# jsappl/DeepPreconditioning

Hardware: NVIDIA B200
Metric: pcg_solves_per_sec (higher is better)
Workload: dtype f64

## Files before the change

deeppreconditioning_b200/_lib.py:

```python

from __future__ import annotations

import ctypes as C
import os
from pathlib import Path

import torch

LIB_PATH = Path(os.environ.get("DPCG_LIB") or Path(__file__).resolve().parent / "lib" / "libdpcg.so")

DP_OK = 0
DP_ERR_STRUCTURE = 5
DP_ERR_TIMEOUT = 6

PRECOND_IDENTITY, PRECOND_JACOBI, PRECOND_MULTIPLY, PRECOND_SOLVE, PRECOND_CSR = range(5)
ENGINE_FUSED, ENGINE_STEPPED = 0, 1
ASSEMBLE_TRIL, ASSEMBLE_TRIL_T, ASSEMBLE_SYMMETRISE = 0, 1, 2

_p = C.c_void_p
_i32 = C.c_int32
_i64 = C.c_int64


class PcgSystem(C.Structure):

    _fields_ = [(name, _i32) for name in (
        "n", "precond", "a_nnz", "m_nnz", "mt_nnz", "fwd_nchunks", "bwd_nchunks",
        "fwd_max_level_chunks", "bwd_max_level_chunks", "solve_algorithm")] + [(name, _p) for name in (
            "a_rowptr", "a_col", "a_val", "m_rowptr", "m_col", "m_val", "mt_rowptr", "mt_col", "mt_val",
            "dinv", "fwd_plan", "bwd_plan",
            "fwd_ls_rowptr", "fwd_ls_col", "fwd_ls_val", "fwd_ls_perm", "fwd_ls_level",
            "bwd_ls_rowptr", "bwd_ls_col", "bwd_ls_val", "bwd_ls_perm", "bwd_ls_level",
            "b", "x", "work", "iters_out", "res_out", "history", "coef",
            "a_col16", "a_val32", "a_tile_base", "m_col16", "m_val32", "m_tile_base",
            "mt_col16", "mt_val32", "mt_tile_base")]


class TrsvSystem(C.Structure):

    _fields_ = [("n", _i32), ("upper", _i32), ("max_level_chunks", _i32), ("reserved", _i32), ("nchunks", _i64)] + [
        (name, _p) for name in ("rowptr", "col", "val", "plan", "b", "x")]


class TrsvLsSystem(C.Structure):

    _fields_ = [("n", _i32), ("nnz", _i32), ("upper", _i32), ("flags", _i32)] + [
        (name, _p) for name in ("rowptr_p", "col_p", "val_p", "perm", "level_sorted", "b", "x")]


class PcgParams(C.Structure):

    _fields_ = [("rtol", C.c_double), ("max_iter", _i32), ("engine", _i32), ("check_every", _i32), ("reserved", _i32)]


class SpconvLayer(C.Structure):

    _fields_ = [("nout", _i64), ("ntaps", _i32), ("cin", _i32), ("cout", _i32), ("reserved", _i32)] + [
        (name, _p) for name in ("src", "in_", "weight", "bias", "slope", "head_weight", "head_bias", "indices", "out")]


class DpcgError(RuntimeError):
    pass


_SIGNATURES = {
    "dp_version": (C.c_int, []),
    "dp_status_string": (C.c_char_p, [C.c_int]),
    "dp_last_cuda_error": (C.c_char_p, []),
    "dp_device_info": (C.c_int, [C.POINTER(C.c_int)] * 3),
    "dp_csr_from_coo_workspace_bytes": (C.c_size_t, [_i32, _i64]),
    "dp_csr_from_coo": (C.c_int, [_p, _p, _i64, _i32, _i32, _i32, _p, _p, _p, _p, _p, _p, C.c_size_t, _p]),
    "dp_csr_transpose_workspace_bytes": (C.c_size_t, [_i32, _i32]),
    "dp_csr_transpose": (C.c_int, [_i32, _i32, _p, _p, _p, _p, _p, _p, _p, C.c_size_t, _p]),
    "dp_csr_inv_diagonal": (C.c_int, [_i32, _p, _p, _p, _p, _p, _p]),
    "dp_csr_aat_nnz": (C.c_int, [_i32, _p, _p, _p, _p, _p, _p]),
    "dp_spmv_csr_f64": (C.c_int, [_i32, _i32, _p, _p, _p, _p, _p, _p]),
    "dp_csr_pack_tile_rows": (_i32, []),
    "dp_csr_pack": (C.c_int, [_i32, _i32, _p, _p, _p, _p, _p, _p, _p, _p]),
    "dp_spmv_csr_packed_f64": (C.c_int, [_i32, _i32, _p, _p, _p, _p, _p, _p, _p]),
    "dp_coo_spmv_batch_f32": (C.c_int, [_p, _p, _i64, _i32, _i32, _p, _i32, _p, _p]),
    "dp_sptrsv_analyse_workspace_bytes": (C.c_size_t, [_i32]),
    "dp_sptrsv_analyse": (C.c_int, [_i32, _p, _p, _i32, _p, _p, _p, _p, _p, _p, C.c_size_t, _p]),
    "dp_sptrsv_plan_chunks": (_i64, [_i32, _p]),
    "dp_sptrsv_plan_sizes_workspace_bytes": (C.c_size_t, [_i32]),
    "dp_sptrsv_plan_sizes": (C.c_int, [_i32, _p, _p, _p, _p, _p, C.c_size_t, _p]),
    "dp_sptrsv_plan_build": (C.c_int, [_i32, _i32, _p, _p, _p, _p, _i64, _p]),
    "dp_sptrsv_workspace_bytes": (C.c_size_t, []),
    "dp_sptrsv_solve_f64": (C.c_int, [_i32, _p, _p, _p, _i32, _p, _i64, _i32, _p, _p, _p, _p, C.c_size_t, _p]),
    "dp_sptrsv_batch_workspace_bytes": (C.c_size_t, [_i32]),
    "dp_sptrsv_solve_batch_f64": (C.c_int, [C.POINTER(TrsvSystem), _i32, _p, _p, C.c_size_t, _p]),
    "dp_sptrsv_permute_workspace_bytes": (C.c_size_t, [_i32]),
    "dp_sptrsv_permute": (C.c_int, [_i32, _i32, _p, _p, _p, _p, _p, _p, _p, _p, _p, _p, _p, C.c_size_t, _p]),
    "dp_sptrsv_ls_limits": (None, [_p]),
    "dp_sptrsv_ls_workspace_bytes": (C.c_size_t, [_i32]),
    "dp_sptrsv_ls_solve_batch_f64": (C.c_int, [C.POINTER(TrsvLsSystem), _i32, _p, C.c_size_t, _p]),
    "dp_sptrsv_ls_prepare": (C.c_int, [C.POINTER(TrsvLsSystem), _i32, _p, C.c_size_t, _p]),
    "dp_sptrsv_ls_launch": (C.c_int, [_i32, _p, C.c_size_t, _p]),
    "dp_sptrsv_ts_prepare": (C.c_int, [C.POINTER(TrsvLsSystem), _i32, _p, C.c_size_t, _p]),
    "dp_sptrsv_ts_launch": (C.c_int, [_i32, _i32, _i32, _i32, _i32, _p, _p, _p]),
    "dp_sptrsv_ts_limits": (None, [_p]),
    "dp_sptrsv_ts_workspace_bytes": (C.c_size_t, [C.POINTER(TrsvLsSystem), _i32]),
    "dp_sptrsv_ts_solve_batch_f64": (C.c_int, [C.POINTER(TrsvLsSystem), _i32, _p, _p, C.c_size_t, _p]),
    "dp_ic0_f64": (C.c_int, [_i32, _p, _p, _p, _p, _p, _i64, _i32, _p, _p, C.c_size_t, _p]),
    "dp_icholt_host": (C.c_int, [_i32, _p, _p, _p, _i32, C.c_double, _p, _p, _p, _i64, _p]),
    "dp_spconv_sort_workspace_bytes": (C.c_size_t, [_i32, _i32]),
    "dp_spconv_sort_sites": (C.c_int, [_p, _i64, _i32, _i32, _i32, _p, _p, _p, _p, _p, C.c_size_t, _p]),
    "dp_spconv_rules_workspace_bytes": (C.c_size_t, [_i32, _i32, _i32]),
    "dp_spconv_rules_count": (C.c_int, [_p, _p, _i32, _i32, _i32, _i32, _i32, _p, _p, C.c_size_t, _p]),
    "dp_spconv_rules_fill": (C.c_int, [_p, _p, _p, _i32, _i32, _i32, _i32, _i32, _p, _p, _p, _p, _p]),
    "dp_spconv_layer_f32": (C.c_int, [C.POINTER(SpconvLayer), _p]),
    "dp_pcg_work_doubles": (_i64, [_i32]),
    "dp_pcg_workspace_bytes": (C.c_size_t, [_i32]),
    "dp_debug_pcg_trace": (C.c_int, [_p, _i32, _p, _i32]),
    "dp_debug_pipe_trace": (C.c_int, [_p, _i32, _i32]),
    "dp_pcg_solve_f64": (C.c_int, [C.POINTER(PcgSystem), _i32, C.POINTER(PcgParams), _p, _p, C.c_size_t, _p]),
}

EXPORTED_SYMBOLS = tuple(_SIGNATURES)

_lib = None


def lib() -> C.CDLL:
    global _lib
    if _lib is None:
        if not LIB_PATH.exists():
            raise DpcgError(
                f"{LIB_PATH} is missing: build it with `python -m deeppreconditioning_b200.build` "
                "(nvcc, sm_100a). deeppreconditioning_b200 has no CPU fallback."
            )
        handle = C.CDLL(str(LIB_PATH))
        for name, (restype, argtypes) in _SIGNATURES.items():
            fn = getattr(handle, name)
            fn.restype, fn.argtypes = restype, argtypes
        _lib = handle
    return _lib


def check(status: int, what: str = "") -> None:
    if status != DP_OK:
        l = lib()
        msg = l.dp_status_string(status).decode()
        if status == 4:
            msg += f" ({l.dp_last_cuda_error().decode()})"
        raise DpcgError(f"libdpcg {what}: {msg}")


def ptr(t: torch.Tensor | None) -> int | None:
    if t is None:
        return None
    if not t.is_cuda:
        raise DpcgError("libdpcg takes device pointers: got a CPU tensor (no CPU fallback)")
    if not t.is_contiguous():
        raise DpcgError("libdpcg needs contiguous tensors")
    return t.data_ptr()


def stream_ptr(device=None) -> int:
    return torch.cuda.current_stream(device).cuda_stream


def device_info() -> dict:
    sm, ctas, l2 = C.c_int(), C.c_int(), C.c_int()
    check(lib().dp_device_info(C.byref(sm), C.byref(ctas), C.byref(l2)), "dp_device_info")
    return {"sm_count": sm.value, "pcg_ctas_per_sm": ctas.value, "l2_bytes": l2.value}


def raise_on_flag(flag: torch.Tensor, what: str) -> None:
    value = int(flag.item())
    if value:
        raise DpcgError(f"libdpcg {what}: device flag {value} ({lib().dp_status_string(value).decode()})")
```

deeppreconditioning_b200/cg.py:

```python

from __future__ import annotations

import ctypes
import time
from dataclasses import dataclass, field

import torch

from . import _lib
from .precond import Identity, _Operator, as_operator, fill_packed
from .sparse import CsrMatrix, _workspace, as_csr, pack_many

_ENGINES = {"fused": _lib.ENGINE_FUSED, "stepped": _lib.ENGINE_STEPPED}


@dataclass
class PcgResult:
    seconds: float
    iterations: int
    info: int
    x_hat: torch.Tensor
    res: float
    history: list = field(default_factory=list)
    alphas: list = field(default_factory=list)
    betas: list = field(default_factory=list)

    @property
    def kappa(self) -> float:
        from .spectrum import kappa_estimate

        return kappa_estimate(self.alphas, self.betas) if self.alphas else float("nan")


def stopping_criterion(_, rk, b):
    return torch.inner(rk, rk) / torch.inner(b, b)


class PcgBatch:

    def __init__(self, systems, rtol: float = 1e-8, max_iter: int = 1024, engine: str = "fused",
                 check_every: int = 32, history: bool = False, device=None, pack: bool = True) -> None:
        if not systems:
            raise ValueError("empty batch")
        self.device = torch.device(device) if device is not None else None
        self.rtol, self.max_iter = float(rtol), int(max_iter)
        self.params = _lib.PcgParams(self.rtol, self.max_iter, _ENGINES[engine], int(check_every), 0)
        self.entries = []
        lib = _lib.lib()
        for item in systems:
            A, b, M = item[0], item[1], item[2]
            x0 = item[3] if len(item) > 3 else None
            A = as_csr(A, self.device)
            if self.device is None:
                self.device = A.device
            if A.device != self.device:
                raise _lib.DpcgError("all systems of a batch must live on one device")
            M = as_operator(M, self.device)
            n = A.n
            b_dev = b.detach().to(device=self.device, dtype=torch.float64).contiguous()
            if b_dev.shape != (n,):
                raise ValueError(f"right-hand side has shape {tuple(b_dev.shape)}, expected ({n},)")
            f64 = dict(dtype=torch.float64, device=self.device)
            x = (x0.detach().to(**f64).clone() if x0 is not None else torch.zeros(n, **f64)).contiguous()
            work = torch.empty(lib.dp_pcg_work_doubles(n), **f64)
            hist = torch.full((self.max_iter + 1,), float("nan"), **f64) if history else None
            coef = torch.full((2 * (self.max_iter + 1),), float("nan"), **f64) if history else None
            self.entries.append(dict(A=A, M=M, b=b_dev, x=x, work=work, hist=hist, coef=coef, out_device=b.device))
        nsys = len(self.entries)
        if any(getattr(e["M"], "tile_stream", False) for e in self.entries):
            self.params = _lib.PcgParams(self.rtol, self.max_iter, _ENGINES["stepped"], min(int(check_every), 8), 0)
        solve_mode = any(e["M"].precond == _lib.PRECOND_SOLVE for e in self.entries)
        if pack and engine == "fused" and not solve_mode:
            pack_many([m for e in self.entries for m in [e["A"], *e["M"].stream_matrices()]])
        self.iters = torch.full((nsys,), -1, dtype=torch.int32, device=self.device)
        self.res = torch.full((nsys,), float("nan"), dtype=torch.float64, device=self.device)
        self.flag = torch.zeros(1, dtype=torch.int32, device=self.device)
        self.ws = _workspace(lib.dp_pcg_workspace_bytes(nsys), self.device)
        self.descs = (_lib.PcgSystem * nsys)()
        for i, e in enumerate(self.entries):
            d, A = self.descs[i], e["A"]
            d.n, d.a_nnz = A.n, A.nnz
            d.a_rowptr, d.a_col, d.a_val = _lib.ptr(A.rowptr), _lib.ptr(A.col), _lib.ptr(A.val)
            fill_packed(d, "a", A)
            e["M"].fill(d)
            if not pack:
                for tag in ("a", "m", "mt"):
                    for name in ("col16", "val32", "tile_base"):
                        setattr(d, f"{tag}_{name}", None)
            d.b, d.x, d.work = _lib.ptr(e["b"]), _lib.ptr(e["x"]), _lib.ptr(e["work"])
            d.iters_out = self.iters.data_ptr() + 4 * i
            d.res_out = self.res.data_ptr() + 8 * i
            d.history = _lib.ptr(e["hist"])
            d.coef = _lib.ptr(e["coef"])

    def __len__(self) -> int:
        return len(self.entries)

    def reset(self, x0s=None) -> None:
        for i, e in enumerate(self.entries):
            if x0s is not None and x0s[i] is not None:
                e["x"].copy_(x0s[i])
            else:
                e["x"].zero_()
        self.iters.fill_(-1)
        self.res.fill_(float("nan"))

    def solve(self) -> None:
        with torch.cuda.device(self.device):
            _lib.check(_lib.lib().dp_pcg_solve_f64(self.descs, len(self.entries), ctypes.byref(self.params),
                                                   _lib.ptr(self.flag), _lib.ptr(self.ws), self.ws.numel(),
                                                   _lib.stream_ptr(self.device)), "dp_pcg_solve_f64")

    def results(self, seconds: float = 0.0) -> list[PcgResult]:
        _lib.raise_on_flag(self.flag, "dp_pcg_solve_f64")
        iters, res = self.iters.cpu().tolist(), self.res.cpu().tolist()
        xs = []
        for e in self.entries:
            if e["out_device"].type == "cpu":
                host = torch.empty(e["x"].shape, dtype=torch.float64, pin_memory=True)
                host.copy_(e["x"], non_blocking=True)
                xs.append(host)
            else:
                xs.append(e["x"].to(e["out_device"]))
        torch.cuda.synchronize(self.device)
        out = []
        for i, e in enumerate(self.entries):
            hist = e["hist"][: iters[i] + 1].cpu().tolist() if e["hist"] is not None and iters[i] >= 0 else []
            alphas, betas = [], []
            if e["coef"] is not None and iters[i] > 0:
                c = e["coef"][: 2 * iters[i]].cpu().view(-1, 2)
                alphas, betas = c[:, 0].tolist(), c[:, 1].tolist()
                betas[0] = 0.0
            out.append(PcgResult(seconds, int(iters[i]), 0, xs[i], float(res[i]), hist, alphas, betas))
        return out


def pcg_solve_batch(systems, rtol: float = 1e-8, max_iter: int = 1024, engine: str = "fused", check_every: int = 32,
                    history: bool = False, device=None, pack: bool = True) -> list[PcgResult]:
    batch = PcgBatch(systems, rtol, max_iter, engine, check_every, history, device, pack)
    torch.cuda.synchronize(batch.device)
    start = time.perf_counter()
    batch.solve()
    torch.cuda.synchronize(batch.device)
    return batch.results(time.perf_counter() - start)


def pcg_solve(A, b, M=None, x0=None, rtol: float = 1e-8, max_iter: int = 1024, engine: str = "fused",
              check_every: int = 32, history: bool = False, pack: bool = True) -> PcgResult:
    return pcg_solve_batch([(A, b, M, x0)], rtol, max_iter, engine, check_every, history, pack=pack)[0]


def preconditioned_conjugate_gradient(A, b: torch.Tensor, M, x0=None, x_true=None, rtol=1e-8, max_iter=1024):
    result = pcg_solve(A, b, M, x0, rtol, max_iter)
    return result.seconds, result.iterations, 0


def conjugate_gradient(A, b, x0=None, x_true=None, rtol=1e-8, max_iter=1024):
    result = pcg_solve(A, b, Identity(), x0, rtol, max_iter, history=True)
    f64 = torch.float64
    tail = torch.zeros(len(result.history), dtype=f64)
    if x_true is not None and result.history:
        A_dev = as_csr(A)
        e = result.x_hat.to(device=A_dev.device, dtype=f64) - x_true.to(device=A_dev.device, dtype=f64)
        last = float(torch.inner(e, A_dev.matvec(e)))
        b64 = b.detach().to(f64)
        bb = float(torch.inner(b64, b64))
        drops = torch.tensor([a * r * bb for a, r in zip(result.alphas, result.history[:-1])], dtype=f64)
        tail[:-1] = torch.flip(torch.cumsum(torch.flip(drops, [0]), 0), [0])
        tail = tail + last
    errors = [(tail[k], torch.tensor(r, dtype=f64)) for k, r in enumerate(result.history)]
    return errors, result.x_hat
```

deeppreconditioning_b200/csrc/pcg.cu:

```cuda
#include <stdlib.h>

#include <vector>

#include "sptrsv.cuh"
#include "trsv_ts.cuh"
#include "tilepipe.cuh"
#include "trsv_ls.cuh"

namespace dp {

int trsv_lookahead();
int pipe_trace_read_spmv(uint64_t* out_host, int capacity);

struct SysDev {
    int n, precond, ntiles;
    int rearm_t;
    int fwd_look, bwd_look;
    CsrView A, M, Mt;
    const double* dinv;
    const int* fwd_plan;
    const int* bwd_plan;
    LsFactor fwd_ls, bwd_ls;
    const double* b;
    double* x;
    double* r[2];
    double* p[2];
    double* z[2];
    double* ap;
    double* t;
    double* part_rr;
    double* part_pap;
    double* part_bb;
    double* part_rz[2];
    double* scal;
    int* iters_out;
    double* res_out;
    double* history;
    double* coef;
};

struct Ctx {
    const SysDev* sys;
    int* state;
    const int* tile_ofs;
    const int* fwd_ofs;
    const int* bwd_ofs;
    int* act_sys[2];
    int* act_ofs[2];
    int* act_meta;
    int nsys, total_tiles, total_fwd, total_bwd;
    int pw_fwd, pw_bwd;
    int has_multiply, has_solve, has_ls;
    int keep_l2;
    double rtol;
    int max_iter;
    unsigned long long* word;
    int* n_done;
    int* flag;
    long long* trace;
    int trace_cap;
};

#ifndef DPCG_ROUND_TILES
#define DPCG_ROUND_TILES 64
#endif
constexpr int kMaxRoundTiles = DPCG_ROUND_TILES;
#ifndef DPCG_APPLY2_UNROLL
#define DPCG_APPLY2_UNROLL kPipeUnroll
#endif
constexpr int kApply2Unroll = DPCG_APPLY2_UNROLL;
#ifndef DPCG_PHASEA_UNROLL
#define DPCG_PHASEA_UNROLL 3
#endif
#ifndef DPCG_APPLY1_UNROLL
#define DPCG_APPLY1_UNROLL 3
#endif
constexpr int kPhaseAUnroll = DPCG_PHASEA_UNROLL;
constexpr int kApply1Unroll = DPCG_APPLY1_UNROLL;
enum Table { TAB_A = 0, TAB_P1 = 1, TAB_P2 = 2 };

struct Smem {
    PipeShared pipe;
    TileDesc tab[3][kMaxRoundTiles];
    double scratch[2][3 * kWarpsPerBlock];
    TileRed red;
    LsShared ls;
    double scratch2[3 * kWarpsPerBlock];
    SysDev sys;
    int sys_id;
    int tab_ver[3], tab_ga[3], tab_gb[3];
    int scan[kWarpsPerBlock + 1];
    int trace_pos;
    int bcast;
};

static_assert(sizeof(SysDev) % 8 == 0, "SysDev is copied as 8-byte words");
static_assert(sizeof(Smem) <= (233472 / 2) - 1024, "two CTAs per SM: 228 KB of shared memory, 1 KB reserved per CTA");

enum Phase { PH_INIT = 0, PH_A = 1, PH_APPLY1 = 2, PH_APPLY2 = 3, PH_FWD = 4, PH_BWD = 5, PH_DOTRZ = 6 };

__device__ __forceinline__ void trace(const Ctx& ctx, Smem& sm, int label) {
    if (ctx.trace_cap > 0 && blockIdx.x == 0 && threadIdx.x == 0) {
        const int i = sm.trace_pos;
        if (i < ctx.trace_cap) {
            ctx.trace[2 * i] = label;
            ctx.trace[2 * i + 1] = clock64();
            sm.trace_pos = i + 1;
        }
    }
}

__device__ __forceinline__ const SysDev& load_sys(const Ctx& ctx, int s, Smem& sm) {
    if (sm.sys_id != s) {
        __syncthreads();
        const unsigned long long* src = reinterpret_cast<const unsigned long long*>(ctx.sys + s);
        unsigned long long* dst = reinterpret_cast<unsigned long long*>(&sm.sys);
        for (int i = threadIdx.x; i < (int)(sizeof(SysDev) / 8); i += kBlock) dst[i] = __ldg(src + i);
        if (threadIdx.x == 0) sm.sys_id = s;
        __syncthreads();
    }
    return sm.sys;
}

__device__ __forceinline__ int find_segment(const int* ofs, int count, int g) {
    int lo = 0, hi = count;
    while (hi - lo > 1) {
        const int mid = (lo + hi) >> 1;
        if (__ldcg(ofs + mid) <= g) lo = mid; else hi = mid;
    }
    return lo;
}

struct Scal {
    int sys = -1;
    bool active = false;
    double v = 0.0;
};

template <class P>
__device__ __forceinline__ void phase_init(const Ctx& ctx, const SysDev& S, const TileDesc& d, int rs, int re,
                                           Smem& sm, P& pipe) {
    const int tile = d.ltile;
    const int row = tile * kTileRows + threadIdx.x;
    const double ax = pipe.tile_spmv(d, rs, re, GatherPlain{S.x}, true);
    double bb[1] = {0.0};
    if (row < S.n && row_thread()) {
        const double bi = S.b[row];
        S.r[1][row] = __dsub_rn(bi, ax);
        S.p[0][row] = 0.0;
        bb[0] = __dmul_rn(bi, bi);
        if (S.precond == DP_PRECOND_SOLVE) {
            st_relaxed_u64(S.z[0] + row, kPending);
            st_relaxed_u64(S.t + row, kPending);
        }
    }
    if (threadIdx.x == 0 && tile == 0) ctx.state[d.sys] = 0;
    double* part_bb = S.part_bb;
    auto write = [part_bb, tile](const double (&v)[1]) { part_bb[tile] = v[0]; };
    if (d.ce > d.cs) {
        tile_reduce_async<1>(bb, sm.red, pipe, write);
    } else {
        tile_reduce<1>(bb, sm.scratch, pipe);
        if (threadIdx.x == 0) write(bb);
    }
}

template <bool kCheckState, class P>
__device__ __forceinline__ void phase_a(const Ctx& ctx, const SysDev& S, const TileDesc& d, int rs, int re, int k,
                                        Smem& sm, Scal& sc, P& pipe) {
    const int s = d.sys, tile = d.ltile;
    const int row = tile * kTileRows + threadIdx.x;
    const bool valid = row < S.n && row_thread();
    const double* z = S.z[k & 1];
    const double* po = S.p[k & 1];
    double zr = 0.0, pr = 0.0;
    if (valid) zr = z[row], pr = po[row];
    if (pipe.ghost) {
        if (d.span > 0) prefetch_columns(z, d.base, d.span), prefetch_columns(po, d.base, d.span);
        else prefetch_tile_rows(z, tile, S.n), prefetch_tile_rows(po, tile, S.n);
    }
    if (sc.sys != s) {
        sc.sys = s;
        sc.active = false;
        bool done = false;
        if (kCheckState) done = __syncthreads_or(threadIdx.x == 0 ? ld_relaxed_s32(ctx.state + s) : 0) != 0;
        if (!done) {
            double v[2] = {0.0, 0.0};
            const double* prr = S.part_rr;
            const double* prz = S.part_rz[k & 1];
            if (row_thread()) {
                for (int i = threadIdx.x; i < S.ntiles; i += kBlock) {
                    v[0] = __dadd_rn(v[0], __ldcg(prr + i));
                    v[1] = __dadd_rn(v[1], __ldcg(prz + i));
                }
            }
            const double bb = __ldcg(S.scal + 2);
            const double rz_prev = k > 0 ? __ldcg(S.scal + ((k - 1) & 1)) : 1.0;
            block_sum_n<2>(v, sm.scratch2);
            const double res = v[0] / bb;
            const bool finished = (res < ctx.rtol) || (k >= ctx.max_iter);
            sc.active = !finished;
            sc.v = k > 0 ? v[1] / rz_prev : 0.0;
            if (tile == 0 && threadIdx.x == 0) {
                if (S.history) S.history[k] = res;
                if (finished) {
                    *S.iters_out = k;
                    *S.res_out = res;
                    ctx.state[s] = 1;
                    atomicAdd(ctx.n_done, 1);
                    atomicAdd(ctx.word, kDoneUnit);
                } else {
                    S.scal[k & 1] = v[1];
                    if (S.coef) S.coef[2 * k + 1] = sc.v;
                }
            }
        }
    }
    if (!sc.active) {
        pipe.tile_skip(d);
        return;
    }
    double* pn = S.p[(k + 1) & 1];
    const double ap = pipe.template tile_spmv<kPhaseAUnroll>(d, rs, re, GatherZBetaP{z, po, sc.v}, true);
    double pap[1] = {0.0};
    if (valid) {
        const double pi = __dadd_rn(zr, __dmul_rn(sc.v, pr));
        pn[row] = pi;
        S.ap[row] = ap;
        pap[0] = __dmul_rn(ap, pi);
        if (S.precond == DP_PRECOND_SOLVE) st_relaxed_u64(S.z[(k + 1) & 1] + row, kPending);
    }
    double* part_pap = S.part_pap;
    auto write = [part_pap, tile](const double (&v)[1]) { part_pap[tile] = v[0]; };
    if (d.ce > d.cs) {
        tile_reduce_async<1>(pap, sm.red, pipe, write);
    } else {
        tile_reduce<1>(pap, sm.scratch, pipe);
        if (threadIdx.x == 0) write(pap);
    }
}

template <bool kInit, class P>
__device__ __forceinline__ void phase_apply1(const Ctx& ctx, const SysDev& S, const TileDesc& d, int rs, int re, int k,
                                             Smem& sm, Scal& sc, P& pipe) {
    const int s = d.sys, tile = d.ltile;
    const int row = tile * kTileRows + threadIdx.x;
    const bool valid = row < S.n && row_thread();
    const double* ro = S.r[k & 1];
    double* rnw = S.r[(k + 1) & 1];
    const double* pn = S.p[(k + 1) & 1];
    double* zn = S.z[(k + 1) & 1];
    const int precond = S.precond;
    double r_old = 0.0, ap_i = 0.0, x_i = 0.0, p_i = 0.0, dinv_i = 0.0;
    if (pipe.ghost) {
        if (d.span > 0) {
            prefetch_columns(ro, d.base, d.span);
            if (!kInit) prefetch_columns(S.ap, d.base, d.span);
        }
        prefetch_tile_rows(ro, tile, S.n);
        if (!kInit) prefetch_tile_rows(S.ap, tile, S.n), prefetch_tile_rows(S.x, tile, S.n), prefetch_tile_rows(pn, tile, S.n);
    }
    if (valid) {
        r_old = ro[row];
        if (!kInit) ap_i = S.ap[row], x_i = S.x[row], p_i = pn[row];
        if (precond == DP_PRECOND_JACOBI) dinv_i = __ldg(S.dinv + row);
    }
    if (sc.sys != s) {
        sc.sys = s;
        sc.active = kInit || ld_relaxed_s32(ctx.state + s) == 0;
        sc.v = 0.0;
        if (!kInit && sc.active) {
            sc.v = __ldcg(S.scal + (k & 1)) / block_reduce_array(S.part_pap, S.ntiles, sm.scratch2);
            if (tile == 0 && threadIdx.x == 0 && S.coef) S.coef[2 * k] = sc.v;
        }
    }
    if (!sc.active) {
        pipe.tile_skip(d);
        return;
    }
    const double a = sc.v;

    double rn = 0.0;
    if (valid) {
        rn = kInit ? r_old : __dsub_rn(r_old, __dmul_rn(a, ap_i));
        rnw[row] = rn;
        if (!kInit) S.x[row] = __dadd_rn(x_i, __dmul_rn(a, p_i));
    }
    double zi = 0.0;
    bool have_z = true;
    switch (precond) {
        case DP_PRECOND_IDENTITY:
            zi = rn;
            break;
        case DP_PRECOND_JACOBI:
            zi = __dmul_rn(dinv_i, rn);
            break;
        case DP_PRECOND_CSR:
            zi = kInit ? pipe.tile_spmv(d, rs, re, GatherWork{ro}, true)
                       : pipe.template tile_spmv<kApply1Unroll>(d, rs, re, GatherRMinusAAp{ro, S.ap, a}, true);
            break;
        case DP_PRECOND_MULTIPLY: {
            const double ti = kInit ? pipe.tile_spmv(d, rs, re, GatherWork{ro}, true)
                                    : pipe.template tile_spmv<kApply1Unroll>(d, rs, re, GatherRMinusAAp{ro, S.ap, a}, true);
            if (valid) S.t[row] = ti;
            have_z = false;
            break;
        }
        default:
            have_z = false;
            break;
    }
    if (have_z && valid) zn[row] = zi;
    double v[3] = {__dmul_rn(rn, rn), __dmul_rn(rn, zi), __dmul_rn(zi, zi)};
    double* part_rr = S.part_rr;
    double* part_rz = S.part_rz[(k + 1) & 1];
    auto write = [part_rr, part_rz, tile, have_z](const double (&w)[3]) {
        if (!kInit) part_rr[tile] = w[0];
        if (have_z) {
            part_rz[tile] = w[1];
            if (kInit) part_rr[tile] = w[2];
        }
    };
    if (d.ce > d.cs) {
        tile_reduce_async<3>(v, sm.red, pipe, write);
    } else {
        tile_reduce<3>(v, sm.scratch, pipe);
        if (threadIdx.x == 0) write(v);
    }
    if (kInit && tile == 0) {
        const double bb = block_reduce_array(S.part_bb, S.ntiles, sm.scratch2);
        if (threadIdx.x == 0) S.scal[2] = bb;
    }
}

template <bool kInit, class P>
__device__ __forceinline__ void phase_apply2(const Ctx& ctx, const SysDev& S, const TileDesc& d, int rs, int re, int k,
                                             Smem& sm, Scal& sc, P& pipe) {
    const int s = d.sys, tile = d.ltile;
    if (sc.sys != s) {
        sc.sys = s;
        sc.active = S.precond == DP_PRECOND_MULTIPLY && (kInit || ld_relaxed_s32(ctx.state + s) == 0);
    }
    if (!sc.active) {
        pipe.tile_skip(d);
        return;
    }
    const int row = tile * kTileRows + threadIdx.x;
    const bool valid = row < S.n && row_thread();
    double rn = 0.0;
    if (valid) rn = S.r[(k + 1) & 1][row];
    if (pipe.ghost) {
        prefetch_tile_rows(S.r[(k + 1) & 1], tile, S.n);
        if (d.span > 0) prefetch_columns(S.t, d.base, d.span);
    }
    const double zi = pipe.template tile_spmv<kApply2Unroll>(d, rs, re, GatherWork{S.t}, true);
    if (valid) S.z[(k + 1) & 1][row] = zi;
    double v[2] = {__dmul_rn(rn, zi), __dmul_rn(zi, zi)};
    double* part_rr = S.part_rr;
    double* part_rz = S.part_rz[(k + 1) & 1];
    auto write = [part_rr, part_rz, tile](const double (&w)[2]) {
        part_rz[tile] = w[0];
        if (kInit) part_rr[tile] = w[1];
    };
    if (d.ce > d.cs) {
        tile_reduce_async<2>(v, sm.red, pipe, write);
    } else {
        tile_reduce<2>(v, sm.scratch, pipe);
        if (threadIdx.x == 0) write(v);
    }
}

template <bool kInit, class P>
__device__ __forceinline__ void phase_dotrz(const Ctx& ctx, const SysDev& S, const TileDesc& d, int k, Smem& sm, Scal& sc,
                                            P& pipe) {
    const int s = d.sys, tile = d.ltile;
    if (sc.sys != s) {
        sc.sys = s;
        sc.active = S.precond == DP_PRECOND_SOLVE && (kInit || ld_relaxed_s32(ctx.state + s) == 0);
    }
    if (!sc.active) return;
    const int row = tile * kTileRows + threadIdx.x;
    double rn = 0.0, zi = 0.0;
    if (row < S.n && row_thread()) {
        rn = S.r[(k + 1) & 1][row];
        zi = S.z[(k + 1) & 1][row];
        if (S.rearm_t) st_relaxed_u64(S.t + row, kPending);
    }
    double v[2] = {__dmul_rn(rn, zi), __dmul_rn(zi, zi)};
    tile_reduce<2>(v, sm.scratch, pipe);
    if (threadIdx.x == 0) {
        S.part_rz[(k + 1) & 1][tile] = v[0];
        if (kInit) S.part_rr[tile] = v[1];
    }
}

template <bool kUpper>
__device__ __noinline__ void trsv_level_stream_outlined(const LsFactor* F, const double* rhs, double* x,
                                                        unsigned char* stage_bytes, LsShared* ls) {
    trsv_level_stream<kUpper, kLsStagesFused>(*F, rhs, x, stage_bytes, *ls);
}

template <bool kUpper, bool kInit>
__device__ __forceinline__ void phase_trsv_ls(const Ctx& ctx, int k, Smem& sm) {
    for (int s = blockIdx.x; s < ctx.nsys; s += gridDim.x) {
        const SysDev* S = ctx.sys + s;
        if (S->precond != DP_PRECOND_SOLVE) continue;
        const LsFactor F = kUpper ? S->bwd_ls : S->fwd_ls;
        if (!F.rowptr) continue;
        if (!kInit && ld_relaxed_s32(ctx.state + s) != 0) continue;
        const double* rhs = kUpper ? S->t : S->r[(k + 1) & 1];
        double* x = kUpper ? S->z[(k + 1) & 1] : S->t;
        trsv_level_stream_outlined<kUpper>(&F, rhs, x, sm.pipe.bytes, &sm.ls);
    }
}

template <bool kUpper, bool kInit>
__device__ __forceinline__ bool phase_trsv(const Ctx& ctx, int k, const Smem& sm) {
    const int pw = kUpper ? ctx.pw_bwd : ctx.pw_fwd;
    const int gw = (threadIdx.x >> 5) * gridDim.x + blockIdx.x;
    if (gw >= pw) return true;
    const int* ofs = kUpper ? ctx.bwd_ofs : ctx.fwd_ofs;
    const AbortCtl ctl{ctx.word, ctx.flag};
    const int nsys = ctx.nsys;
    const int wps = pw >= nsys ? pw / nsys : 1;
    const int local = pw >= nsys ? gw / nsys : 0;
    if (local >= wps) return true;
    for (int s = pw >= nsys ? gw % nsys : gw; s < nsys; s += pw) {
        const SysDev& S = (sm.sys_id == s) ? sm.sys : ctx.sys[s];
        if (S.precond != DP_PRECOND_SOLVE) continue;
        if ((kUpper ? S.bwd_ls.rowptr : S.fwd_ls.rowptr) != nullptr) continue;
        if (!kInit && ld_relaxed_s32(ctx.state + s) != 0) continue;
        const long long nchunks = __ldg(ofs + s + 1) - __ldg(ofs + s);
        bool ok;
        if (kUpper)
            ok = sptrsv_stream<true>(S.Mt, S.bwd_plan, local, wps, nchunks, S.bwd_look, RhsConsume{S.t}, S.z[(k + 1) & 1], ctl);
        else
            ok = sptrsv_stream<false>(S.M, S.fwd_plan, local, wps, nchunks, S.fwd_look, RhsPlain{S.r[(k + 1) & 1]}, S.t, ctl);
        if (!ok) return false;
    }
    return true;
}

template <int kPhase, bool kInit, bool kCheckState, class P>
__device__ __forceinline__ void run_tile(const Ctx& ctx, const SysDev& S, const TileDesc& d, int rs, int re, int k,
                                         Smem& sm, Scal& sc, P& pipe) {
    if (kPhase == PH_INIT) phase_init(ctx, S, d, rs, re, sm, pipe);
    if (kPhase == PH_A) phase_a<kCheckState>(ctx, S, d, rs, re, k, sm, sc, pipe);
    if (kPhase == PH_APPLY1) phase_apply1<kInit>(ctx, S, d, rs, re, k, sm, sc, pipe);
    if (kPhase == PH_APPLY2) phase_apply2<kInit>(ctx, S, d, rs, re, k, sm, sc, pipe);
    if (kPhase == PH_DOTRZ) phase_dotrz<kInit>(ctx, S, d, k, sm, sc, pipe);
}

template <int kTab, bool kPacked>
__device__ __forceinline__ void build_table(const Ctx& ctx, int cur, int ga, int gb, Smem& sm) {
    const int count = __ldcg(ctx.act_meta + 2 * cur);
    const int* asys = ctx.act_sys[cur];
    const int* aofs = ctx.act_ofs[cur];
    for (int i = threadIdx.x; i < gb - ga; i += kBlock) {
        const int g = ga + i;
        const int seg = count == 1 ? 0 : find_segment(aofs, count, g);
        const int s = __ldcg(asys + seg);
        const int lt = g - __ldcg(aofs + seg);
        const SysDev* S = ctx.sys + s;
        const int precond = S->precond;
        CsrView M{nullptr, nullptr, nullptr, 0, 0};
        if (kTab == TAB_A) M = S->A;
        if (kTab == TAB_P1 && precond == DP_PRECOND_MULTIPLY) M = S->Mt;
        if (kTab == TAB_P1 && precond == DP_PRECOND_CSR) M = S->M;
        if (kTab == TAB_P2 && precond == DP_PRECOND_MULTIPLY) M = S->M;
        TileDesc d;
        tile_desc_fill<kPacked>(d, M, lt);
        d.sys = s;
        sm.tab[kTab][i] = d;
    }
}

template <int kTab, bool kPacked>
__device__ __forceinline__ void ensure_table(const Ctx& ctx, int cur, int ver, int ga, int gb, Smem& sm) {
    if (sm.tab_ver[kTab] == ver && sm.tab_ga[kTab] == ga && sm.tab_gb[kTab] == gb) return;
    __syncthreads();
    build_table<kTab, kPacked>(ctx, cur, ga, gb, sm);
    if (threadIdx.x == 0) sm.tab_ver[kTab] = ver, sm.tab_ga[kTab] = ga, sm.tab_gb[kTab] = gb;
    __syncthreads();
}

template <int kPhase, bool kInit, bool kCheckState, class P>
__device__ __forceinline__ void run_tiles(const Ctx& ctx, int k, int cur, int ver, int total, Smem& sm, P& pipe,
                                          int next_tab = -1) {
    constexpr int kTab = kPhase == PH_APPLY1 ? TAB_P1 : kPhase == PH_APPLY2 ? TAB_P2 : TAB_A;
    constexpr bool kStream = kPhase != PH_DOTRZ;
    const int quot = total / (int)gridDim.x, rem = total % (int)gridDim.x;
    const int g0 = (int)blockIdx.x * quot + min((int)blockIdx.x, rem), g1 = g0 + quot + ((int)blockIdx.x < rem ? 1 : 0);
    Scal sc;
#ifdef DPCG_PIPE_TRACE
    pipe.tr_phase = kPhase;
#endif
    for (int ga = g0; ga < g1; ga += kMaxRoundTiles) {
        const int gb = min(g1, ga + kMaxRoundTiles);
        ensure_table<kTab, P::kIsPacked>(ctx, cur, ver, ga, gb, sm);
        const TileDesc* tab = sm.tab[kTab];
        if (kStream) {
            if (!pipe.begin_resume(tab, gb - ga, kTab)) {
                pipe.drain_early();
                pipe.begin(tab, gb - ga);
            }
        }
        for (int i = 0; i < gb - ga; ++i) {
            const TileDesc& d = tab[i];
            const SysDev& S = load_sys(ctx, d.sys, sm);
            int rs = 0, re = 0;
            if (kStream) tile_row_extent(d, rs, re);
            run_tile<kPhase, kInit, kCheckState>(ctx, S, d, rs, re, k, sm, sc, pipe);
#ifdef DPCG_PIPE_TRACE
            pipe.tr_mark(5);
#endif
        }
    }
    if (next_tab >= 0 && g1 > g0 && g1 - g0 <= kMaxRoundTiles && sm.tab_ver[next_tab] == ver &&
        sm.tab_ga[next_tab] == g0 && sm.tab_gb[next_tab] == g1)
        pipe.begin_early(sm.tab[next_tab], g1 - g0, next_tab);
}

__device__ __forceinline__ void rebuild_active(const Ctx& ctx, int cur, Smem& sm) {
    const int count = __ldcg(ctx.act_meta + 2 * cur);
    const int* asys = ctx.act_sys[cur];
    const int* aofs = ctx.act_ofs[cur];
    int* nsys_out = ctx.act_sys[cur ^ 1];
    int* nofs_out = ctx.act_ofs[cur ^ 1];
    int carry_n = 0, carry_t = 0;
    for (int i0 = 0; i0 < count; i0 += kBlock) {
        const int i = i0 + threadIdx.x;
        int s = -1, alive = 0, nt = 0;
        if (i < count && row_thread()) {
            s = __ldcg(asys + i);
            alive = ld_relaxed_s32(ctx.state + s) == 0;
            nt = alive ? __ldcg(aofs + i + 1) - __ldcg(aofs + i) : 0;
        }
        int tot_n, tot_t;
        const int pos = block_exclusive_scan_int(alive, &tot_n, sm.scan);
        const int tofs = block_exclusive_scan_int(nt, &tot_t, sm.scan);
        if (alive) {
            nsys_out[carry_n + pos] = s;
            nofs_out[carry_n + pos] = carry_t + tofs;
        }
        carry_n += tot_n;
        carry_t += tot_t;
    }
    if (threadIdx.x == 0) {
        nofs_out[carry_n] = carry_t;
        ctx.act_meta[2 * (cur ^ 1)] = carry_n;
        ctx.act_meta[2 * (cur ^ 1) + 1] = carry_t;
    }
}

template <bool kInit, bool kSolve, class P>
__device__ __forceinline__ bool apply_preconditioner(const Ctx& ctx, int k, int cur, int ver, int total, GridBarrier& bar,
                                                     Smem& sm, P& pipe, bool list_stays) {
    const int tab_a = list_stays ? (int)TAB_A : -1;
    run_tiles<PH_APPLY1, kInit, false>(ctx, k, cur, ver, total, sm, pipe,
                                       ctx.has_multiply ? (int)TAB_P2 : (kSolve ? -1 : tab_a));
    trace(ctx, sm, 8 * PH_APPLY1 + 1);
    if (bar.sync() < 0) return false;
    trace(ctx, sm, 8 * PH_APPLY1 + 2);
    if (ctx.has_multiply) {
        run_tiles<PH_APPLY2, kInit, false>(ctx, k, cur, ver, total, sm, pipe, kSolve ? -1 : tab_a);
        trace(ctx, sm, 8 * PH_APPLY2 + 1);
        if (bar.sync() < 0) return false;
        trace(ctx, sm, 8 * PH_APPLY2 + 2);
    }
    if (kSolve) {
        if (ctx.has_ls) phase_trsv_ls<false, kInit>(ctx, k, sm);
        const bool f = phase_trsv<false, kInit>(ctx, k, sm);
        if (bar.sync() < 0 || !f) return false;
        if (ctx.has_ls) phase_trsv_ls<true, kInit>(ctx, k, sm);
        const bool b = phase_trsv<true, kInit>(ctx, k, sm);
        if (bar.sync() < 0 || !b) return false;
        run_tiles<PH_DOTRZ, kInit, false>(ctx, k, cur, ver, total, sm, pipe, tab_a);
        if (bar.sync() < 0) return false;
    }
    return true;
}

template <class P>
__device__ __forceinline__ Smem& smem_init(unsigned char* raw, P& pipe) {
    Smem& sm = *reinterpret_cast<Smem*>(raw);
    if (threadIdx.x == 0) {
        sm.sys_id = -1, sm.trace_pos = 0;
        sm.tab_ver[0] = sm.tab_ver[1] = sm.tab_ver[2] = 0;
        for (int i = 0; i < kRedRing; ++i) sm.red.count[i] = 0;
        sm.ls.init();
    }
    pipe.init(sm.pipe.bytes, &sm.pipe.bar);
    return sm;
}

constexpr int kFusedThreadsPacked = kPackProducerWarp ? kBlock + kWarp : kBlock;
template <bool kSolve, bool kPacked>
__global__ void __launch_bounds__(kPacked ? kFusedThreadsPacked : kBlock, 2) pcg_fused_kernel(Ctx ctx) {
    extern __shared__ __align__(16) unsigned char smem_raw[];
    typename std::conditional<kPacked, PipePacked, Pipe>::type pipe;
    Smem& sm = smem_init(smem_raw, pipe);
    pipe.keep_l2 = ctx.keep_l2;
    GridBarrier bar{ctx.word, ctx.flag, &sm.bcast, 0u, gridDim.x};
    int cur = 0;
    int ver = 1;
    int done_built = 0;
    int total = ctx.total_tiles;
    run_tiles<PH_INIT, false, false>(ctx, -1, cur, ver, total, sm, pipe, TAB_P1);
    if (bar.sync() < 0) return;
    if (!apply_preconditioner<true, kSolve>(ctx, -1, cur, ver, total, bar, sm, pipe, true)) return;
    for (int k = 0; k <= ctx.max_iter; ++k) {
        trace(ctx, sm, 8 * PH_A + 0);
        run_tiles<PH_A, false, false>(ctx, k, cur, ver, total, sm, pipe, TAB_P1);
        trace(ctx, sm, 8 * PH_A + 1);
        const int done = bar.sync();
        trace(ctx, sm, 8 * PH_A + 2);
        if (done < 0) return;
        if (done >= ctx.nsys) {
            pipe.drain_early();
            break;
        }
        const bool rebuild = done != done_built;
        if (rebuild && blockIdx.x == 0) rebuild_active(ctx, cur, sm);
        if (!apply_preconditioner<false, kSolve>(ctx, k, cur, ver, total, bar, sm, pipe, !rebuild)) return;
        if (rebuild) {
            cur ^= 1, done_built = done, ++ver;
            total = __ldcg(ctx.act_meta + 2 * cur + 1);
        }
    }
}

template <int kPhase, bool kInit>
__global__ void __launch_bounds__(kBlock, 2) pcg_phase_kernel(Ctx ctx, int k) {
    extern __shared__ __align__(16) unsigned char smem_raw[];
    Pipe pipe;
    Smem& sm = smem_init(smem_raw, pipe);
    pipe.keep_l2 = ctx.keep_l2;
    if (kPhase == PH_FWD) {
        if (ctx.has_ls) phase_trsv_ls<false, kInit>(ctx, k, sm);
        phase_trsv<false, kInit>(ctx, k, sm);
    } else if (kPhase == PH_BWD) {
        if (ctx.has_ls) phase_trsv_ls<true, kInit>(ctx, k, sm);
        phase_trsv<true, kInit>(ctx, k, sm);
    } else {
        run_tiles<kPhase, kInit, true>(ctx, k, 0, 1, ctx.total_tiles, sm, pipe);
    }
}

__device__ __forceinline__ double tile_sum(double v, double (*scratch)[kWarpsPerBlock], int& flip) {
    const int lane = threadIdx.x & 31, warp = threadIdx.x >> 5;
    double* sc = scratch[flip];
    flip ^= 1;
    v = warp_sum(v);
    if (lane == 0) sc[warp] = v;
    __syncthreads();
    return half_warp_sum(sc[lane & (kWarpsPerBlock - 1)]);
}

struct LeanCursor {
    int g, g1, s, lo, hi;
    __device__ __forceinline__ void init(const Ctx& ctx) {
        const int total = ctx.total_tiles;
        const int quot = total / (int)gridDim.x, rem = total % (int)gridDim.x;
        g = (int)blockIdx.x * quot + min((int)blockIdx.x, rem);
        g1 = g + quot + ((int)blockIdx.x < rem ? 1 : 0);
        s = g < g1 ? find_segment(ctx.tile_ofs, ctx.nsys, g) : 0;
        lo = __ldg(ctx.tile_ofs + s), hi = __ldg(ctx.tile_ofs + s + 1);
    }
    __device__ __forceinline__ bool advance(const Ctx& ctx) {
        bool changed = false;
        while (g >= hi) ++s, lo = hi, hi = __ldg(ctx.tile_ofs + s + 1), changed = true;
        return changed;
    }
};

template <bool kInit>
__global__ void __launch_bounds__(kBlock, 3) solve_apply1_kernel(Ctx ctx, int k) {
    __shared__ double scratch[2][kWarpsPerBlock];
    __shared__ double scratch2[kWarpsPerBlock];
    int flip = 0;
    LeanCursor cur;
    cur.init(ctx);
    bool fresh = true, active = false;
    double a = 0.0;
    const double *ro = nullptr, *ap = nullptr, *pn = nullptr;
    double *rnw = nullptr, *x = nullptr, *part_rr = nullptr;
    int n = 0;
    for (; cur.g < cur.g1; ++cur.g) {
        if (cur.advance(ctx) || fresh) {
            fresh = false;
            const SysDev* S = ctx.sys + cur.s;
            n = S->n;
            ro = S->r[k & 1], rnw = S->r[(k + 1) & 1], pn = S->p[(k + 1) & 1], ap = S->ap, x = S->x, part_rr = S->part_rr;
            active = kInit || ld_relaxed_s32(ctx.state + cur.s) == 0;
            a = 0.0;
            if (!kInit && active) a = __ldcg(S->scal + (k & 1)) / block_reduce_array(S->part_pap, S->ntiles, scratch2);
        }
        const int tile = cur.g - cur.lo;
        if (!active) continue;
        const int row = tile * kTileRows + threadIdx.x;
        double rn = 0.0;
        if (row < n) {
            const double r_old = ro[row];
            if (kInit) {
                rn = r_old;
            } else {
                const double ap_i = ap[row], x_i = x[row], p_i = pn[row];
                rn = __dsub_rn(r_old, __dmul_rn(a, ap_i));
                x[row] = __dadd_rn(x_i, __dmul_rn(a, p_i));
            }
            rnw[row] = rn;
        }
        if (!kInit) {
            const double rr = tile_sum(__dmul_rn(rn, rn), scratch, flip);
            if (threadIdx.x == 0) part_rr[tile] = rr;
        }
        if (tile == 0) {
            const SysDev* S = ctx.sys + cur.s;
            if (!kInit && threadIdx.x == 0 && S->coef) S->coef[2 * k] = a;
            if (kInit) {
                const double bb = block_reduce_array(S->part_bb, S->ntiles, scratch2);
                if (threadIdx.x == 0) S->scal[2] = bb;
            }
        }
    }
}

template <bool kInit>
__global__ void __launch_bounds__(kBlock, 3) solve_dotrz_kernel(Ctx ctx, int k) {
    __shared__ double scratch[2][kWarpsPerBlock];
    int flip = 0;
    LeanCursor cur;
    cur.init(ctx);
    bool fresh = true, active = false;
    const double *rn = nullptr, *zn = nullptr;
    double *t = nullptr, *part_rz = nullptr, *part_rr = nullptr;
    int n = 0, rearm = 0;
    for (; cur.g < cur.g1; ++cur.g) {
        if (cur.advance(ctx) || fresh) {
            fresh = false;
            const SysDev* S = ctx.sys + cur.s;
            n = S->n, rearm = S->rearm_t;
            rn = S->r[(k + 1) & 1], zn = S->z[(k + 1) & 1], t = S->t, part_rz = S->part_rz[(k + 1) & 1], part_rr = S->part_rr;
            active = kInit || ld_relaxed_s32(ctx.state + cur.s) == 0;
        }
        const int tile = cur.g - cur.lo;
        if (!active) continue;
        const int row = tile * kTileRows + threadIdx.x;
        double ri = 0.0, zi = 0.0;
        if (row < n) {
            ri = rn[row], zi = zn[row];
            if (rearm) st_relaxed_u64(t + row, kPending);
        }
        const double rz = tile_sum(__dmul_rn(ri, zi), scratch, flip);
        if (threadIdx.x == 0) part_rz[tile] = rz;
        if (kInit) {
            const double zz = tile_sum(__dmul_rn(zi, zi), scratch, flip);
            if (threadIdx.x == 0) part_rr[tile] = zz;
        }
    }
}

static inline int64_t pad32(int64_t v) { return (v + 31) / 32 * 32; }
static inline int ntiles_of(int n) { return (n + kTileRows - 1) / kTileRows; }
constexpr int kTraceCap = 4096;

struct WsLayout {
    size_t word, n_done, meta, sys, state, tile_ofs, fwd_ofs, bwd_ofs, act_sys[2], act_ofs[2], trace, ts_word, ts_sys[4], total;
};
static WsLayout ws_layout(int nsys) {
    WsLayout w{};
    size_t off = 0;
    auto take = [&](size_t bytes) { size_t at = off; off += align_up(bytes, 256); return at; };
    const size_t ints = sizeof(int) * ((size_t)nsys + 1);
    w.word = take(8);
    w.n_done = take(4);
    w.meta = take(16);
    w.sys = take(sizeof(SysDev) * (size_t)nsys);
    w.state = take(ints);
    w.tile_ofs = take(ints);
    w.fwd_ofs = take(ints);
    w.bwd_ofs = take(ints);
    for (int i = 0; i < 2; ++i) w.act_sys[i] = take(ints), w.act_ofs[i] = take(ints);
    w.trace = take(sizeof(long long) * 2 * kTraceCap);
    w.ts_word = take(8);
    for (int i = 0; i < 4; ++i) w.ts_sys[i] = take(sizeof(TsSysDev) * (size_t)nsys);
    w.total = off;
    return w;
}

template <class Kernel>
static int allow_smem(Kernel kernel) {
    return allow_dynamic_smem((const void*)kernel, sizeof(Smem));
}

template <int kPhase, bool kInit>
static int launch_phase(const Ctx& ctx, int k, int grid, bool cooperative, cudaStream_t s) {
    int st = allow_smem(pcg_phase_kernel<kPhase, kInit>);
    if (st != DP_OK) return st;
    if (cooperative) {
        Ctx c = ctx;
        void* args[] = {&c, &k};
        DP_CUDA(cudaLaunchCooperativeKernel((const void*)pcg_phase_kernel<kPhase, kInit>, dim3(grid), dim3(kBlock), args,
                                            sizeof(Smem), s));
    } else {
        pcg_phase_kernel<kPhase, kInit><<<grid, kBlock, sizeof(Smem), s>>>(ctx, k);
        DP_LAUNCH_CHECK();
    }
    return DP_OK;
}

struct TsPhases {
    const TsSysDev* fwd[2];
    const TsSysDev* bwd[2];
    int nsys, max_tiles, nmax;
    bool short_rows;
    bool all_solve;
    unsigned long long* word;
};

template <bool kInit>
static int launch_lean(bool dotrz, const Ctx& ctx, int k, cudaStream_t s) {
    const void* kernel = dotrz ? (const void*)solve_dotrz_kernel<kInit> : (const void*)solve_apply1_kernel<kInit>;
    int grid = coop_grid(kernel, kBlock, 0);
    if (grid > ctx.total_tiles) grid = ctx.total_tiles;
    if (dotrz)
        solve_dotrz_kernel<kInit><<<grid, kBlock, 0, s>>>(ctx, k);
    else
        solve_apply1_kernel<kInit><<<grid, kBlock, 0, s>>>(ctx, k);
    DP_LAUNCH_CHECK();
    return DP_OK;
}

template <bool kInit>
static int launch_apply(const Ctx& ctx, int k, int tile_grid, int coop, const TsPhases* ts, cudaStream_t s) {
    int st;
    const bool lean = ts != nullptr && ts->all_solve;
    if (lean) {
        if ((st = launch_lean<kInit>(false, ctx, k, s)) != DP_OK) return st;
    } else if ((st = launch_phase<PH_APPLY1, kInit>(ctx, k, tile_grid, false, s)) != DP_OK) return st;
    if (ctx.has_multiply && (st = launch_phase<PH_APPLY2, kInit>(ctx, k, tile_grid, false, s)) != DP_OK) return st;
    if (ctx.has_solve) {
        if (ts) {
            const int par = (k + 1) & 1;
            if ((st = ts_solve_launch(ts->fwd[par], ts->nsys, ts->max_tiles, ts->nmax, ts->short_rows, false, ts->word, ctx.flag, s)) != DP_OK) return st;
            if ((st = ts_solve_launch(ts->bwd[par], ts->nsys, ts->max_tiles, ts->nmax, ts->short_rows, false, ts->word, ctx.flag, s)) != DP_OK) return st;
        } else {
            if ((st = launch_phase<PH_FWD, kInit>(ctx, k, coop, true, s)) != DP_OK) return st;
            if ((st = launch_phase<PH_BWD, kInit>(ctx, k, coop, true, s)) != DP_OK) return st;
        }
        if (lean) {
            if ((st = launch_lean<kInit>(true, ctx, k, s)) != DP_OK) return st;
        } else if ((st = launch_phase<PH_DOTRZ, kInit>(ctx, k, tile_grid, false, s)) != DP_OK) return st;
    }
    return DP_OK;
}

}

using namespace dp;

extern "C" {

int64_t dp_pcg_work_doubles(int32_t n) {
    if (n < 0) return -1;
    return 8 * pad32(n) + 5 * pad32(ntiles_of(n)) + 32;
}

size_t dp_pcg_workspace_bytes(int32_t nsys) { return ws_layout(nsys < 0 ? 0 : nsys).total; }

int dp_device_info(int* sm_count_host, int* pcg_ctas_per_sm_host, int* l2_bytes_host) {
    int dev = 0, sms = 0, l2 = 0;
    DP_CUDA(cudaGetDevice(&dev));
    DP_CUDA(cudaDeviceGetAttribute(&sms, cudaDevAttrMultiProcessorCount, dev));
    DP_CUDA(cudaDeviceGetAttribute(&l2, cudaDevAttrL2CacheSize, dev));
    if (sm_count_host) *sm_count_host = sms;
    if (l2_bytes_host) *l2_bytes_host = l2;
    if (pcg_ctas_per_sm_host) {
        if (allow_smem(pcg_fused_kernel<false, false>) != DP_OK) return DP_ERR_CUDA;
        *pcg_ctas_per_sm_host = coop_grid((const void*)pcg_fused_kernel<false, false>, kBlock, sizeof(Smem)) / (sms > 0 ? sms : 1);
    }
    return DP_OK;
}

int dp_debug_pcg_trace(const void* workspace, int32_t nsys, int64_t* out_host, int32_t capacity) {
    if (!workspace || !out_host || capacity <= 0 || nsys <= 0) return DP_ERR_INVALID;
    const WsLayout lay = ws_layout(nsys);
    const int cap = capacity < kTraceCap ? capacity : kTraceCap;
    DP_CUDA(cudaMemcpy(out_host, static_cast<const char*>(workspace) + lay.trace, sizeof(long long) * 2 * (size_t)cap,
                       cudaMemcpyDeviceToHost));
    return DP_OK;
}

int dp_debug_pipe_trace(uint64_t* out_host, int32_t capacity, int32_t unit) {
#ifdef DPCG_PIPE_TRACE
    if (!out_host || capacity <= 0) return DP_ERR_INVALID;
    if (unit == 1) return dp::pipe_trace_read_spmv(out_host, capacity);
    const int cap = capacity < kPipeTraceCap ? capacity : kPipeTraceCap;
    for (int w = 0; w < 2; ++w)
        DP_CUDA(cudaMemcpyFromSymbol(out_host + (size_t)w * capacity, g_pipe_trace, sizeof(unsigned long long) * (size_t)cap,
                                     sizeof(unsigned long long) * (size_t)w * kPipeTraceCap, cudaMemcpyDeviceToHost));
    return DP_OK;
#else
    (void)out_host, (void)capacity, (void)unit;
    return DP_ERR_INVALID;
#endif
}

int dp_pcg_solve_f64(const dp_pcg_system_t* systems_host, int32_t nsys, const dp_pcg_params_t* params_host,
                     int32_t* flag_out, void* workspace, size_t workspace_bytes, void* stream) {
    if (!systems_host || nsys <= 0 || !params_host || !flag_out || !workspace) return DP_ERR_INVALID;
    if (params_host->max_iter < 0) return DP_ERR_INVALID;
    if (!aligned16(workspace)) return DP_ERR_ALIGNMENT;
    const WsLayout lay = ws_layout(nsys);
    if (workspace_bytes < lay.total) return DP_ERR_WORKSPACE;
    cudaStream_t s = (cudaStream_t)stream;
    char* ws = static_cast<char*>(workspace);

    std::vector<SysDev> sys((size_t)nsys);
    std::vector<int> tile_ofs((size_t)nsys + 1, 0), fwd_ofs((size_t)nsys + 1, 0), bwd_ofs((size_t)nsys + 1, 0);
    std::vector<int> ident((size_t)nsys + 1, 0);
    int has_multiply = 0, has_solve = 0, has_ls = 0, n_solve = 0, n_ts = 0;
    bool packed = true;
    long long working_set_bytes = 0, matrix_entries = 0;
    long long sum_fwd_lvl = 0, sum_bwd_lvl = 0;
    std::vector<TsSysDev> ts_sys[4];
    std::vector<int> ts_owner;
    bool ts_short = true;
    for (int i = 0; i < nsys; ++i) {
        const dp_pcg_system_t& u = systems_host[i];
        if (u.n <= 0 || !u.a_rowptr || !u.a_col || !u.a_val || !u.b || !u.x || !u.work || !u.iters_out || !u.res_out)
            return DP_ERR_INVALID;
        if (!aligned16(u.a_col) || !aligned16(u.a_val) || !aligned16(u.work)) return DP_ERR_ALIGNMENT;
        SysDev d{};
        d.n = u.n;
        d.precond = u.precond;
        d.ntiles = ntiles_of(u.n);
        d.A = CsrView{u.a_rowptr, u.a_col, u.a_val, u.n, u.a_nnz, u.a_col16, u.a_val32, u.a_tile_base};
        d.M = CsrView{u.m_rowptr, u.m_col, u.m_val, u.n, u.m_nnz, u.m_col16, u.m_val32, u.m_tile_base};
        d.Mt = CsrView{u.mt_rowptr, u.mt_col, u.mt_val, u.n, u.mt_nnz, u.mt_col16, u.mt_val32, u.mt_tile_base};
        {
            auto has_pack = [](const CsrView& V) { return V.col16 && V.val32 && V.tbase && aligned16(V.col16) && aligned16(V.val32); };
            if (!has_pack(d.A)) packed = false;
            if ((u.precond == DP_PRECOND_MULTIPLY || u.precond == DP_PRECOND_CSR) && !has_pack(d.M)) packed = false;
            if (u.precond == DP_PRECOND_MULTIPLY && !has_pack(d.Mt)) packed = false;
            if (u.precond == DP_PRECOND_SOLVE) packed = false;
        }
        d.dinv = u.dinv;
        d.fwd_plan = u.fwd_plan;
        d.bwd_plan = u.bwd_plan;
        d.fwd_ls = LsFactor{nullptr, nullptr, nullptr, nullptr, nullptr, 0, 0};
        d.bwd_ls = d.fwd_ls;
        const bool tile_stream = u.precond == DP_PRECOND_SOLVE && (u.solve_algorithm & DP_SOLVE_TILE_STREAM) != 0;
        if (tile_stream && !(u.solve_algorithm & DP_SOLVE_SHORT_ROWS)) ts_short = false;
        if (u.precond == DP_PRECOND_SOLVE) ++n_solve;
        if (tile_stream) {
            if (!u.fwd_ls_rowptr || !u.fwd_ls_col || !u.fwd_ls_val || !u.bwd_ls_rowptr || !u.bwd_ls_col || !u.bwd_ls_val)
                return DP_ERR_INVALID;
            if (!aligned16(u.fwd_ls_rowptr) || !aligned16(u.fwd_ls_col) || !aligned16(u.fwd_ls_val) ||
                !aligned16(u.bwd_ls_rowptr) || !aligned16(u.bwd_ls_col) || !aligned16(u.bwd_ls_val))
                return DP_ERR_ALIGNMENT;
            ++n_ts;
        } else if (u.precond == DP_PRECOND_SOLVE) {
            if (u.fwd_ls_rowptr && u.fwd_ls_col && u.fwd_ls_val) {
                if (!aligned16(u.fwd_ls_col) || !aligned16(u.fwd_ls_val) || !aligned16(u.fwd_ls_rowptr)) return DP_ERR_ALIGNMENT;
                d.fwd_ls = LsFactor{u.fwd_ls_rowptr, u.fwd_ls_col, u.fwd_ls_val, u.fwd_ls_perm, u.fwd_ls_level, u.n, u.m_nnz};
                has_ls = 1;
            }
            if (u.bwd_ls_rowptr && u.bwd_ls_col && u.bwd_ls_val) {
                if (!aligned16(u.bwd_ls_col) || !aligned16(u.bwd_ls_val) || !aligned16(u.bwd_ls_rowptr)) return DP_ERR_ALIGNMENT;
                d.bwd_ls = LsFactor{u.bwd_ls_rowptr, u.bwd_ls_col, u.bwd_ls_val, u.bwd_ls_perm, u.bwd_ls_level, u.n, u.mt_nnz};
                has_ls = 1;
            }
        }
        d.rearm_t = tile_stream || (u.precond == DP_PRECOND_SOLVE && !d.fwd_ls.rowptr && d.bwd_ls.rowptr) ? 1 : 0;
        d.fwd_look = u.fwd_max_level_chunks > 0 ? u.fwd_max_level_chunks : 1;
        d.bwd_look = u.bwd_max_level_chunks > 0 ? u.bwd_max_level_chunks : 1;
        int fwd_chunks = 0, bwd_chunks = 0;
        switch (u.precond) {
            case DP_PRECOND_IDENTITY: break;
            case DP_PRECOND_JACOBI:
                if (!u.dinv) return DP_ERR_INVALID;
                break;
            case DP_PRECOND_CSR:
                if (!u.m_rowptr || !u.m_col || !u.m_val) return DP_ERR_INVALID;
                if (!aligned16(u.m_col) || !aligned16(u.m_val)) return DP_ERR_ALIGNMENT;
                break;
            case DP_PRECOND_SOLVE:
                if (!u.fwd_plan || !u.bwd_plan || u.fwd_nchunks <= 0 || u.bwd_nchunks <= 0) return DP_ERR_INVALID;
                fwd_chunks = u.fwd_nchunks;
                bwd_chunks = u.bwd_nchunks;
                sum_fwd_lvl += u.fwd_max_level_chunks > 0 ? u.fwd_max_level_chunks : (1 << 20);
                sum_bwd_lvl += u.bwd_max_level_chunks > 0 ? u.bwd_max_level_chunks : (1 << 20);
                has_solve = 1;
                [[fallthrough]];
            case DP_PRECOND_MULTIPLY:
                if (!u.m_rowptr || !u.m_col || !u.m_val || !u.mt_rowptr || !u.mt_col || !u.mt_val) return DP_ERR_INVALID;
                if (!aligned16(u.m_col) || !aligned16(u.m_val) || !aligned16(u.mt_col) || !aligned16(u.mt_val))
                    return DP_ERR_ALIGNMENT;
                if (u.precond == DP_PRECOND_MULTIPLY) has_multiply = 1;
                break;
            default: return DP_ERR_INVALID;
        }
        d.b = u.b;
        d.x = u.x;
        const long long entries = (long long)u.a_nnz + (u.precond >= DP_PRECOND_MULTIPLY ? u.m_nnz : 0) +
                                  (u.precond == DP_PRECOND_MULTIPLY || u.precond == DP_PRECOND_SOLVE ? u.mt_nnz : 0);
        matrix_entries += entries;
        working_set_bytes += 12ll * entries + 8ll * 10 * u.n;
        const int64_t np = pad32(u.n), tp = pad32(d.ntiles);
        double* w = u.work;
        d.r[0] = w; d.r[1] = w + np; d.p[0] = w + 2 * np; d.p[1] = w + 3 * np;
        d.z[0] = w + 4 * np;
        d.z[1] = u.precond == DP_PRECOND_SOLVE ? w + 5 * np : d.z[0];
        d.ap = w + 6 * np; d.t = w + 7 * np;
        double* q = w + 8 * np;
        d.part_rr = q; d.part_pap = q + tp; d.part_bb = q + 2 * tp; d.part_rz[0] = q + 3 * tp; d.part_rz[1] = q + 4 * tp;
        d.scal = q + 5 * tp;
        d.iters_out = u.iters_out;
        d.res_out = u.res_out;
        d.history = u.history;
        d.coef = u.coef;
        if (tile_stream) {
            for (int par = 0; par < 2; ++par) {
                TsSysDev f{}, g{};
                f.F = LsFactor{u.fwd_ls_rowptr, u.fwd_ls_col, u.fwd_ls_val, nullptr, nullptr, u.n, u.m_nnz};
                f.b = d.r[par], f.x = d.t, f.upper = 0, f.ntiles = d.ntiles, f.rev = 0;
                f.skip = g.skip = reinterpret_cast<const int*>(ws + lay.state) + i;
                g.F = LsFactor{u.bwd_ls_rowptr, u.bwd_ls_col, u.bwd_ls_val, nullptr, nullptr, u.n, u.mt_nnz};
                g.b = d.t, g.x = d.z[par], g.upper = 1, g.ntiles = d.ntiles, g.rev = 1;
                ts_sys[par].push_back(f);
                ts_sys[2 + par].push_back(g);
            }
            ts_owner.push_back(i);
        }
        sys[(size_t)i] = d;
        ident[(size_t)i] = i;
        tile_ofs[(size_t)i + 1] = tile_ofs[(size_t)i] + d.ntiles;
        fwd_ofs[(size_t)i + 1] = fwd_ofs[(size_t)i] + fwd_chunks;
        bwd_ofs[(size_t)i + 1] = bwd_ofs[(size_t)i] + bwd_chunks;
    }

    if (n_ts && (n_ts != n_solve || params_host->engine != DP_ENGINE_STEPPED)) return DP_ERR_INVALID;
    {
        const char* e = getenv("DPCG_NO_PACK");
        if ((e && e[0] == '1') || params_host->engine != DP_ENGINE_FUSED) packed = false;
    }
    const void* fused = has_solve ? (const void*)pcg_fused_kernel<true, false>
                        : packed  ? (const void*)pcg_fused_kernel<false, true>
                                  : (const void*)pcg_fused_kernel<false, false>;
    if (allow_dynamic_smem(fused, sizeof(Smem)) != DP_OK || allow_smem(pcg_phase_kernel<PH_FWD, false>) != DP_OK) return DP_ERR_CUDA;
    const int fused_threads = (!has_solve && packed) ? kFusedThreadsPacked : kBlock;
    const int coop = coop_grid(fused, fused_threads, sizeof(Smem));
    const int coop_phase = coop_grid((const void*)pcg_phase_kernel<PH_FWD, false>, kBlock, sizeof(Smem));
    auto clamp_pw = [](long long lvl_chunks, int grid) {
        long long pw = (long long)trsv_lookahead() * lvl_chunks;
        if (pw < 32) pw = 32;
        const long long w = (long long)grid * kWarpsPerBlock;
        return (int)(pw > w ? w : pw);
    };

    Ctx ctx{};
    ctx.sys = reinterpret_cast<const SysDev*>(ws + lay.sys);
    ctx.state = reinterpret_cast<int*>(ws + lay.state);
    ctx.tile_ofs = reinterpret_cast<const int*>(ws + lay.tile_ofs);
    ctx.fwd_ofs = reinterpret_cast<const int*>(ws + lay.fwd_ofs);
    ctx.bwd_ofs = reinterpret_cast<const int*>(ws + lay.bwd_ofs);
    for (int i = 0; i < 2; ++i) {
        ctx.act_sys[i] = reinterpret_cast<int*>(ws + lay.act_sys[i]);
        ctx.act_ofs[i] = reinterpret_cast<int*>(ws + lay.act_ofs[i]);
    }
    ctx.act_meta = reinterpret_cast<int*>(ws + lay.meta);
    ctx.nsys = nsys;
    ctx.total_tiles = tile_ofs[(size_t)nsys];
    ctx.total_fwd = fwd_ofs[(size_t)nsys];
    ctx.total_bwd = bwd_ofs[(size_t)nsys];
    ctx.has_multiply = has_multiply;
    ctx.has_solve = has_solve;
    ctx.has_ls = has_ls;
    {
        int dev = 0, l2 = 0;
        DP_CUDA(cudaGetDevice(&dev));
        DP_CUDA(cudaDeviceGetAttribute(&l2, cudaDevAttrL2CacheSize, dev));
        const char* e = getenv("DPCG_KEEP_L2");
        if (packed) working_set_bytes -= matrix_entries * 6;
        ctx.keep_l2 = e ? (e[0] == '1') : (working_set_bytes * 10 < (long long)l2 * 6);
    }
    ctx.rtol = params_host->rtol;
    ctx.max_iter = params_host->max_iter;
    ctx.word = reinterpret_cast<unsigned long long*>(ws + lay.word);
    ctx.n_done = reinterpret_cast<int*>(ws + lay.n_done);
    ctx.flag = flag_out;
    ctx.trace = reinterpret_cast<long long*>(ws + lay.trace);
    const char* tr = getenv("DPCG_TRACE");
    ctx.trace_cap = (tr && tr[0] == '1') ? kTraceCap : 0;

    const int meta[4] = {nsys, ctx.total_tiles, 0, 0};
    DP_CUDA(cudaMemsetAsync(ws + lay.word, 0, 8, s));
    DP_CUDA(cudaMemsetAsync(ws + lay.n_done, 0, 4, s));
    if (ctx.trace_cap) DP_CUDA(cudaMemsetAsync(ws + lay.trace, 0, sizeof(long long) * 2 * kTraceCap, s));
    DP_CUDA(cudaMemcpyAsync(ws + lay.meta, meta, sizeof(meta), cudaMemcpyHostToDevice, s));
    DP_CUDA(cudaMemcpyAsync(ws + lay.sys, sys.data(), sizeof(SysDev) * (size_t)nsys, cudaMemcpyHostToDevice, s));
    const size_t ints = sizeof(int) * ((size_t)nsys + 1);
    DP_CUDA(cudaMemcpyAsync(ws + lay.tile_ofs, tile_ofs.data(), ints, cudaMemcpyHostToDevice, s));
    DP_CUDA(cudaMemcpyAsync(ws + lay.fwd_ofs, fwd_ofs.data(), ints, cudaMemcpyHostToDevice, s));
    DP_CUDA(cudaMemcpyAsync(ws + lay.bwd_ofs, bwd_ofs.data(), ints, cudaMemcpyHostToDevice, s));
    DP_CUDA(cudaMemcpyAsync(ws + lay.act_sys[0], ident.data(), ints, cudaMemcpyHostToDevice, s));
    DP_CUDA(cudaMemcpyAsync(ws + lay.act_ofs[0], tile_ofs.data(), ints, cudaMemcpyHostToDevice, s));

    if (params_host->engine == DP_ENGINE_FUSED) {
        int grid = ctx.total_tiles;
        if (has_solve) {
            const long long want = (long long)trsv_lookahead() * (sum_fwd_lvl > sum_bwd_lvl ? sum_fwd_lvl : sum_bwd_lvl);
            if (want > grid) grid = want > coop ? coop : (int)want;
        }
        if (grid > coop) grid = coop;
        if (grid < 1) grid = 1;
        ctx.pw_fwd = clamp_pw(sum_fwd_lvl, grid);
        ctx.pw_bwd = clamp_pw(sum_bwd_lvl, grid);
        void* args[] = {&ctx};
        DP_CUDA(cudaLaunchCooperativeKernel(fused, dim3(grid), dim3(fused_threads), args, sizeof(Smem), s));
        return DP_OK;
    }
    if (params_host->engine != DP_ENGINE_STEPPED) return DP_ERR_INVALID;

    ctx.pw_fwd = clamp_pw(sum_fwd_lvl, coop_phase);
    ctx.pw_bwd = clamp_pw(sum_bwd_lvl, coop_phase);
    TsPhases ts_phases{};
    const TsPhases* ts = nullptr;
    auto ts_upload = [&](const std::vector<int>& keep) -> int {
        std::vector<TsSysDev> act;
        ts_phases.nsys = (int)keep.size(), ts_phases.max_tiles = 0, ts_phases.nmax = 0;
        for (int q = 0; q < 4; ++q) {
            act.clear();
            for (int idx : keep) act.push_back(ts_sys[q][(size_t)idx]);
            DP_CUDA(cudaMemcpyAsync(ws + lay.ts_sys[q], act.data(), sizeof(TsSysDev) * act.size(), cudaMemcpyHostToDevice, s));
        }
        for (int idx : keep) {
            const TsSysDev& f = ts_sys[0][(size_t)idx];
            if (f.ntiles > ts_phases.max_tiles) ts_phases.max_tiles = f.ntiles;
            if (f.F.n > ts_phases.nmax) ts_phases.nmax = f.F.n;
        }
        return DP_OK;
    };
    std::vector<int> ts_keep;
    if (n_ts) {
        DP_CUDA(cudaMemsetAsync(ws + lay.ts_word, 0, 8, s));
        for (int q = 0; q < n_ts; ++q) ts_keep.push_back(q);
        if (ts_upload(ts_keep) != DP_OK) return DP_ERR_CUDA;
        for (int par = 0; par < 2; ++par) {
            ts_phases.fwd[par] = reinterpret_cast<const TsSysDev*>(ws + lay.ts_sys[par]);
            ts_phases.bwd[par] = reinterpret_cast<const TsSysDev*>(ws + lay.ts_sys[2 + par]);
        }
        ts_phases.short_rows = ts_short;
        ts_phases.all_solve = n_ts == nsys;
        ts_phases.word = reinterpret_cast<unsigned long long*>(ws + lay.ts_word);
        ts = &ts_phases;
    }
    const int tile_grid = ctx.total_tiles < coop * 4 ? ctx.total_tiles : coop * 4;
    const int every = params_host->check_every > 0 ? params_host->check_every : 1;
    int st;
    if ((st = launch_phase<PH_INIT, false>(ctx, -1, tile_grid, false, s)) != DP_OK) return st;
    if ((st = launch_apply<true>(ctx, -1, tile_grid, coop_phase, ts, s)) != DP_OK) return st;
    for (int k = 0; k <= ctx.max_iter; ++k) {
        if ((st = launch_phase<PH_A, false>(ctx, k, tile_grid, false, s)) != DP_OK) return st;
        if (k % every == 0 || k == ctx.max_iter) {
            int done = 0;
            DP_CUDA(cudaMemcpyAsync(&done, ctx.n_done, sizeof(int), cudaMemcpyDeviceToHost, s));
            DP_CUDA(cudaStreamSynchronize(s));
            if (done >= nsys) break;
            if (ts && done > nsys - (int)ts_keep.size()) {
                std::vector<int> state((size_t)nsys);
                DP_CUDA(cudaMemcpyAsync(state.data(), ctx.state, sizeof(int) * (size_t)nsys, cudaMemcpyDeviceToHost, s));
                DP_CUDA(cudaStreamSynchronize(s));
                std::vector<int> keep;
                for (int idx : ts_keep)
                    if (state[(size_t)ts_owner[(size_t)idx]] == 0) keep.push_back(idx);
                if (!keep.empty() && keep.size() < ts_keep.size()) {
                    ts_keep.swap(keep);
                    if (ts_upload(ts_keep) != DP_OK) return DP_ERR_CUDA;
                }
            }
        }
        if ((st = launch_apply<false>(ctx, k, tile_grid, coop_phase, ts, s)) != DP_OK) return st;
    }
    return DP_OK;
}

}
```

deeppreconditioning_b200/csrc/spmv.cu:

```cuda
#include <stdio.h>
#include <stdlib.h>
#include <string.h>

#include <mutex>
#include <vector>

#include "tilepipe.cuh"

namespace dp {

static thread_local char g_cuda_error[256] = "";

const char* set_cuda_error(cudaError_t e) {
    snprintf(g_cuda_error, sizeof(g_cuda_error), "%s: %s", cudaGetErrorName(e), cudaGetErrorString(e));
    return g_cuda_error;
}

constexpr int kSpmvRound = 32;
#ifndef DPCG_SPMV_UNROLL
#define DPCG_SPMV_UNROLL 8
#endif

struct SpmvSmem {
    PipeShared pipe;
    TileDesc tab[kSpmvRound];
};

template <bool kPacked>
__global__ void __launch_bounds__(kBlock, 2)
spmv_csr_kernel(CsrView A, const double* __restrict__ x, double* __restrict__ y) {
    extern __shared__ __align__(16) unsigned char smem_raw[];
    SpmvSmem& sm = *reinterpret_cast<SpmvSmem*>(smem_raw);
    typename std::conditional<kPacked, PipePacked, Pipe>::type pipe;
    pipe.init(sm.pipe.bytes, &sm.pipe.bar);
    const int ntiles = (A.n + kTileRows - 1) / kTileRows;
    const int quot = ntiles / (int)gridDim.x, rem = ntiles % (int)gridDim.x;
    const int g0 = (int)blockIdx.x * quot + min((int)blockIdx.x, rem), g1 = g0 + quot + ((int)blockIdx.x < rem ? 1 : 0);
    const GatherReadOnly gx{x};
    for (int ga = g0; ga < g1; ga += kSpmvRound) {
        const int cnt = min(kSpmvRound, g1 - ga);
        __syncthreads();
        for (int i = threadIdx.x; i < cnt; i += kBlock) {
            TileDesc d;
            tile_desc_fill<kPacked>(d, A, ga + i);
            d.sys = 0;
            sm.tab[i] = d;
        }
        __syncthreads();
        pipe.begin(sm.tab, cnt);
        int rs_n, re_n;
        tile_row_extent(sm.tab[0], rs_n, re_n);
        for (int i = 0; i < cnt; ++i) {
            const TileDesc& d = sm.tab[i];
            const int rs = rs_n, re = re_n;
            if (i + 1 < cnt) tile_row_extent(sm.tab[i + 1], rs_n, re_n);
            const double s = pipe.template tile_spmv<DPCG_SPMV_UNROLL>(d, rs, re, gx, true);
            const int row = d.ltile * kTileRows + (int)threadIdx.x;
            if (row < A.n) y[row] = s;
        }
    }
}

__global__ void __launch_bounds__(kBlock)
csr_pack_kernel(int n, const int* __restrict__ rowptr, const int* __restrict__ col, const double* __restrict__ val,
                unsigned short* __restrict__ col16, float* __restrict__ val32, int* __restrict__ tile_base,
                int* __restrict__ status) {
    __shared__ int s_lo[kWarpsPerBlock], s_hi[kWarpsPerBlock];
    const int tile = blockIdx.x;
    const int cs = __ldg(rowptr + min(tile * kTileRows, n)), ce = __ldg(rowptr + min((tile + 1) * kTileRows, n));
    int lo = 0x7fffffff, hi = -1;
    for (int q = cs + (int)threadIdx.x; q < ce; q += kBlock) {
        const int c = __ldg(col + q);
        lo = min(lo, c), hi = max(hi, c);
    }
#pragma unroll
    for (int o = 16; o > 0; o >>= 1) {
        lo = min(lo, __shfl_xor_sync(kFull, lo, o));
        hi = max(hi, __shfl_xor_sync(kFull, hi, o));
    }
    if ((threadIdx.x & 31) == 0) s_lo[threadIdx.x >> 5] = lo, s_hi[threadIdx.x >> 5] = hi;
    __syncthreads();
    lo = s_lo[0], hi = s_hi[0];
#pragma unroll
    for (int w = 1; w < kWarpsPerBlock; ++w) lo = min(lo, s_lo[w]), hi = max(hi, s_hi[w]);
    if (ce == cs) lo = 0, hi = 0;
    int bad = (hi - lo > 65535 || lo < 0) ? 2 : 0;
    if (threadIdx.x == 0) tile_base[2 * tile] = lo, tile_base[2 * tile + 1] = ce > cs ? hi - lo + 1 : 0;
    for (int q = cs + (int)threadIdx.x; q < ce; q += kBlock) {
        const double v = val[q];
        const float f = (float)v;
        if (as_bits((double)f) != as_bits(v)) bad |= 1;
        val32[q] = f;
        col16[q] = (unsigned short)(__ldg(col + q) - lo);
    }
    if (bad) atomicOr(status, bad);
}

__global__ void coo_spmv_batch_kernel(const int* __restrict__ ind, const float* __restrict__ feat, long long nnz,
                                      int nbatch, int n, const float* __restrict__ vec, int transpose,
                                      float* __restrict__ out) {
    for (long long e = blockIdx.x * (long long)blockDim.x + threadIdx.x; e < nnz;
         e += (long long)gridDim.x * blockDim.x) {
        const int b = ind[3 * e], r = ind[3 * e + (transpose ? 2 : 1)], c = ind[3 * e + (transpose ? 1 : 2)];
        if ((unsigned)b < (unsigned)nbatch && (unsigned)r < (unsigned)n && (unsigned)c < (unsigned)n)
            atomicAdd(out + (size_t)b * n + r, feat[e] * vec[(size_t)b * n + c]);
    }
}

namespace {
constexpr int kMaxDevices = 64;
struct KernelEntry {
    int device;
    const void* kernel;
    size_t smem;
    int threads;
    size_t occ_smem;
    int grid;
};
std::mutex g_cache_mutex;
std::vector<KernelEntry> g_kernels;
int g_sm_count[kMaxDevices];

int current_device() {
    int dev = 0;
    return cudaGetDevice(&dev) == cudaSuccess ? dev : 0;
}
KernelEntry& kernel_entry(int dev, const void* kernel) {
    for (KernelEntry& e : g_kernels)
        if (e.device == dev && e.kernel == kernel) return e;
    g_kernels.push_back(KernelEntry{dev, kernel, 0, 0, 0, 0});
    return g_kernels.back();
}
}

int pipe_trace_read_spmv(uint64_t* out_host, int capacity) {
#ifdef DPCG_PIPE_TRACE
    const int cap = capacity < kPipeTraceCap ? capacity : kPipeTraceCap;
    for (int w = 0; w < 2; ++w)
        DP_CUDA(cudaMemcpyFromSymbol(out_host + (size_t)w * capacity, g_pipe_trace, sizeof(unsigned long long) * (size_t)cap,
                                     sizeof(unsigned long long) * (size_t)w * kPipeTraceCap, cudaMemcpyDeviceToHost));
    return DP_OK;
#else
    (void)out_host, (void)capacity;
    return DP_ERR_INVALID;
#endif
}

int sm_count() {
    const int dev = current_device();
    const bool cacheable = dev >= 0 && dev < kMaxDevices;
    if (cacheable && g_sm_count[dev]) return g_sm_count[dev];
    int sms = 0;
    if (cudaDeviceGetAttribute(&sms, cudaDevAttrMultiProcessorCount, dev) != cudaSuccess || sms < 1) return 148;
    if (cacheable) g_sm_count[dev] = sms;
    return sms;
}

int allow_dynamic_smem(const void* kernel, size_t bytes) {
    const int dev = current_device();
    std::lock_guard<std::mutex> lock(g_cache_mutex);
    KernelEntry& e = kernel_entry(dev, kernel);
    if (e.smem >= bytes && e.smem > 0) return DP_OK;
    DP_CUDA(cudaFuncSetAttribute(kernel, cudaFuncAttributeMaxDynamicSharedMemorySize, (int)bytes));
    if (const char* c = getenv("DPCG_CARVEOUT"))
        DP_CUDA(cudaFuncSetAttribute(kernel, cudaFuncAttributePreferredSharedMemoryCarveout, atoi(c)));
    e.smem = bytes;
    e.threads = 0;
    return DP_OK;
}

int coop_grid(const void* kernel, int threads, size_t smem) {
    const int dev = current_device();
    std::lock_guard<std::mutex> lock(g_cache_mutex);
    KernelEntry& e = kernel_entry(dev, kernel);
    if (e.threads == threads && e.occ_smem == smem && e.grid > 0) return e.grid;
    int per_sm = 0;
    if (cudaOccupancyMaxActiveBlocksPerMultiprocessor(&per_sm, kernel, threads, smem) != cudaSuccess || per_sm < 1)
        per_sm = 1;
    int sms = 0;
    if (cudaDeviceGetAttribute(&sms, cudaDevAttrMultiProcessorCount, dev) != cudaSuccess || sms < 1) sms = 148;
    e.threads = threads, e.occ_smem = smem, e.grid = per_sm * sms;
    return e.grid;
}

}

using namespace dp;

extern "C" {

int dp_version(void) { return DP_VERSION; }

const char* dp_status_string(int status) {
    switch (status) {
        case DP_OK: return "ok";
        case DP_ERR_INVALID: return "invalid argument";
        case DP_ERR_ALIGNMENT: return "array not 16-byte aligned";
        case DP_ERR_WORKSPACE: return "workspace too small";
        case DP_ERR_CUDA: return "CUDA runtime error";
        case DP_ERR_STRUCTURE: return "matrix structure violates the contract";
        case DP_ERR_TIMEOUT: return "dependency spin timed out";
        default: return "unknown status";
    }
}

const char* dp_last_cuda_error(void) { return g_cuda_error; }

int dp_spmv_csr_f64(int32_t n, int32_t nnz, const int32_t* rowptr, const int32_t* col, const double* val,
                    const double* x, double* y, void* stream) {
    if (n < 0 || nnz < 0 || !rowptr || !y || (nnz > 0 && (!col || !val || !x))) return DP_ERR_INVALID;
    if (!aligned16(col) || !aligned16(val)) return DP_ERR_ALIGNMENT;
    if (n == 0) return DP_OK;
    if (allow_dynamic_smem((const void*)spmv_csr_kernel<false>, sizeof(SpmvSmem)) != DP_OK) return DP_ERR_CUDA;
    const int tiles = (n + kTileRows - 1) / kTileRows;
    const int resident = 2 * sm_count();
    const int grid = tiles < resident ? tiles : resident;
    CsrView A{rowptr, col, val, n, nnz};
    spmv_csr_kernel<false><<<grid, kBlock, sizeof(SpmvSmem), (cudaStream_t)stream>>>(A, x, y);
    DP_LAUNCH_CHECK();
    return DP_OK;
}

int32_t dp_csr_pack_tile_rows(void) { return kTileRows; }

int dp_csr_pack(int32_t n, int32_t nnz, const int32_t* rowptr, const int32_t* col, const double* val, uint16_t* col16,
                float* val32, int32_t* tile_base, int32_t* status_out, void* stream) {
    if (n < 0 || nnz < 0 || !rowptr || !tile_base || !status_out || (nnz > 0 && (!col || !val || !col16 || !val32)))
        return DP_ERR_INVALID;
    if (!aligned16(col16) || !aligned16(val32)) return DP_ERR_ALIGNMENT;
    if (n == 0) return DP_OK;
    const int tiles = (n + kTileRows - 1) / kTileRows;
    csr_pack_kernel<<<tiles, kBlock, 0, (cudaStream_t)stream>>>(n, rowptr, col, val, col16, val32, tile_base, status_out);
    DP_LAUNCH_CHECK();
    return DP_OK;
}

int dp_spmv_csr_packed_f64(int32_t n, int32_t nnz, const int32_t* rowptr, const uint16_t* col16, const float* val32,
                           const int32_t* tile_base, const double* x, double* y, void* stream) {
    if (n < 0 || nnz < 0 || !rowptr || !y || !tile_base || (nnz > 0 && (!col16 || !val32 || !x))) return DP_ERR_INVALID;
    if (!aligned16(col16) || !aligned16(val32)) return DP_ERR_ALIGNMENT;
    if (n == 0) return DP_OK;
    if (allow_dynamic_smem((const void*)spmv_csr_kernel<true>, sizeof(SpmvSmem)) != DP_OK) return DP_ERR_CUDA;
    const int tiles = (n + kTileRows - 1) / kTileRows;
    const int resident = 2 * sm_count();
    const int grid = tiles < resident ? tiles : resident;
    CsrView A{rowptr, nullptr, nullptr, n, nnz, col16, val32, tile_base};
    spmv_csr_kernel<true><<<grid, kBlock, sizeof(SpmvSmem), (cudaStream_t)stream>>>(A, x, y);
    DP_LAUNCH_CHECK();
    return DP_OK;
}

int dp_coo_spmv_batch_f32(const int32_t* indices, const float* features, int64_t nnz, int32_t nbatch, int32_t n,
                          const float* vec, int32_t transpose, float* out, void* stream) {
    if (nnz < 0 || nbatch < 0 || n < 0 || !out || (nnz > 0 && (!indices || !features || !vec))) return DP_ERR_INVALID;
    cudaStream_t s = (cudaStream_t)stream;
    DP_CUDA(cudaMemsetAsync(out, 0, sizeof(float) * (size_t)nbatch * (size_t)n, s));
    if (nnz == 0) return DP_OK;
    long long blocks = (nnz + 255) / 256;
    if (blocks > sm_count() * 32) blocks = sm_count() * 32;
    coo_spmv_batch_kernel<<<(int)blocks, 256, 0, s>>>(indices, features, nnz, nbatch, n, vec, transpose, out);
    DP_LAUNCH_CHECK();
    return DP_OK;
}

}
```

deeppreconditioning_b200/csrc/tilepipe.cuh:

```cuda
#pragma once

#include <type_traits>

#include "common.cuh"
#include "spmv.cuh"

#ifndef DPCG_PIPE_CAP
#define DPCG_PIPE_CAP 3840
#endif
#ifndef DPCG_PIPE_STAGES
#define DPCG_PIPE_STAGES 2
#endif
#ifndef DPCG_PIPE_UNROLL
#define DPCG_PIPE_UNROLL 4
#endif
#ifndef DPCG_PIPE_EVICT_FIRST
#define DPCG_PIPE_EVICT_FIRST 1
#endif
#ifndef DPCG_PACK_WINDOWS
#define DPCG_PACK_WINDOWS 0
#endif
#ifndef DPCG_PACK_CAP
#if DPCG_PACK_WINDOWS
#define DPCG_PACK_CAP DPCG_PIPE_CAP
#else
#define DPCG_PACK_CAP (2 * DPCG_PIPE_CAP)
#endif
#endif
#ifndef DPCG_PACK_STAGES
#define DPCG_PACK_STAGES DPCG_PIPE_STAGES
#endif
#ifndef DPCG_PACK_PRODUCER_WARP
#define DPCG_PACK_PRODUCER_WARP 1
#endif
#ifndef DPCG_GHOST_PREFETCH
#define DPCG_GHOST_PREFETCH 1
#endif
#ifndef DPCG_GHOST_PREFETCH_GATHER
#define DPCG_GHOST_PREFETCH_GATHER 1
#endif
#ifndef DPCG_PIPE_WAIT_HINT
#define DPCG_PIPE_WAIT_HINT 1000
#endif

namespace dp {

#ifdef DPCG_PIPE_TRACE
constexpr int kPipeTraceCap = 1 << 15;
__device__ unsigned long long g_pipe_trace[2][kPipeTraceCap];
#define DP_PIPE_MARK(label) tr_mark(label)
#else
#define DP_PIPE_MARK(label) ((void)0)
#endif

constexpr int kPipeCap = DPCG_PIPE_CAP;
constexpr int kPipeStages = DPCG_PIPE_STAGES;
constexpr int kPipeUnroll = DPCG_PIPE_UNROLL;
constexpr int kPackCap = DPCG_PACK_CAP;
constexpr int kPackStages = DPCG_PACK_STAGES;
constexpr bool kPackWindows = DPCG_PACK_WINDOWS != 0;
constexpr bool kPackProducerWarp = DPCG_PACK_PRODUCER_WARP != 0;
constexpr int kMaxStages = kPipeStages > kPackStages ? kPipeStages : kPackStages;

__device__ __forceinline__ unsigned smem_u32(const void* p) { return (unsigned)__cvta_generic_to_shared(p); }
__device__ __forceinline__ void mbar_init(unsigned long long* bar, unsigned count) {
    asm volatile("mbarrier.init.shared::cta.b64 [%0], %1;" ::"r"(smem_u32(bar)), "r"(count) : "memory");
}
__device__ __forceinline__ void mbar_fence_init() { asm volatile("fence.mbarrier_init.release.cluster;" ::: "memory"); }
__device__ __forceinline__ void mbar_arrive_expect_tx(unsigned long long* bar, unsigned bytes) {
    asm volatile("mbarrier.arrive.expect_tx.shared::cta.b64 _, [%0], %1;" ::"r"(smem_u32(bar)), "r"(bytes) : "memory");
}
__device__ __forceinline__ bool mbar_try_wait(unsigned long long* bar, unsigned parity) {
    unsigned ok;
    asm volatile(
        "{\n\t.reg .pred p;\n\t"
        "mbarrier.try_wait.parity.shared::cta.b64 p, [%1], %2;\n\t"
        "selp.u32 %0, 1, 0, p;\n\t}"
        : "=r"(ok)
        : "r"(smem_u32(bar)), "r"(parity)
        : "memory");
    return ok != 0;
}
__device__ __forceinline__ bool mbar_try_wait_hint(unsigned long long* bar, unsigned parity, unsigned ns) {
    unsigned ok;
    asm volatile(
        "{\n\t.reg .pred p;\n\t"
        "mbarrier.try_wait.parity.shared::cta.b64 p, [%1], %2, %3;\n\t"
        "selp.u32 %0, 1, 0, p;\n\t}"
        : "=r"(ok)
        : "r"(smem_u32(bar)), "r"(parity), "r"(ns)
        : "memory");
    return ok != 0;
}
__device__ __forceinline__ bool mbar_test_wait(unsigned long long* bar, unsigned parity) {
    unsigned ok;
    asm volatile(
        "{\n\t.reg .pred p;\n\t"
        "mbarrier.test_wait.parity.shared::cta.b64 p, [%1], %2;\n\t"
        "selp.u32 %0, 1, 0, p;\n\t}"
        : "=r"(ok)
        : "r"(smem_u32(bar)), "r"(parity)
        : "memory");
    return ok != 0;
}
__device__ __forceinline__ void mbar_arrive(unsigned long long* bar) {
    asm volatile("mbarrier.arrive.shared::cta.b64 _, [%0];" ::"r"(smem_u32(bar)) : "memory");
}
__device__ __forceinline__ unsigned long long l2_policy_stream() {
    unsigned long long pol;
    asm volatile("createpolicy.fractional.L2::evict_first.b64 %0, 1.0;" : "=l"(pol));
    return pol;
}
__device__ __forceinline__ unsigned long long l2_policy_keep() {
    unsigned long long pol;
    asm volatile("createpolicy.fractional.L2::evict_normal.b64 %0, 1.0;" : "=l"(pol));
    return pol;
}
__device__ __forceinline__ void bulk_g2s(void* dst, const void* src, unsigned bytes, unsigned long long* bar,
                                         unsigned long long policy) {
#if DPCG_PIPE_EVICT_FIRST
    asm volatile(
        "cp.async.bulk.shared::cluster.global.mbarrier::complete_tx::bytes.L2::cache_hint [%0], [%1], %2, [%3], %4;" ::"r"(
            smem_u32(dst)),
        "l"(src), "r"(bytes), "r"(smem_u32(bar)), "l"(policy)
        : "memory");
#else
    asm volatile("cp.async.bulk.shared::cluster.global.mbarrier::complete_tx::bytes [%0], [%1], %2, [%3];" ::"r"(
                     smem_u32(dst)),
                 "l"(src), "r"(bytes), "r"(smem_u32(bar))
                 : "memory");
#endif
}
__device__ __forceinline__ void cp_async_16(void* dst, const void* src) {
    asm volatile("cp.async.cg.shared.global [%0], [%1], 16;" ::"r"(smem_u32(dst)), "l"(src) : "memory");
}
__device__ __forceinline__ void cp_async_mbar_arrive_noinc(unsigned long long* bar) {
    asm volatile("cp.async.mbarrier.arrive.noinc.shared::cta.b64 [%0];" ::"r"(smem_u32(bar)) : "memory");
}
__device__ __forceinline__ void prefetch_tile_rows(const double* v, int tile, int n) {
#if DPCG_GHOST_PREFETCH
    const int row = tile * kTileRows + (int)(threadIdx.x & 31) * 16;
    if (row < n) {
#if DPCG_GHOST_PREFETCH == 1
        asm volatile("prefetch.global.L2 [%0];" ::"l"(v + row));
#else
        asm volatile("prefetch.global.L1 [%0];" ::"l"(v + row));
#endif
    }
#else
    (void)v, (void)tile, (void)n;
#endif
}
__device__ __forceinline__ void prefetch_columns(const double* v, int base, int span) {
#if DPCG_GHOST_PREFETCH && DPCG_GHOST_PREFETCH_GATHER
    for (int c = (int)(threadIdx.x & 31) * 16; c < span; c += 32 * 16) {
#if DPCG_GHOST_PREFETCH == 1
        asm volatile("prefetch.global.L2 [%0];" ::"l"(v + (base & ~15) + c));
#else
        asm volatile("prefetch.global.L1 [%0];" ::"l"(v + (base & ~15) + c));
#endif
    }
#else
    (void)v, (void)base, (void)span;
#endif
}
struct TileDesc {
    const int* rowptr;
    const int* col;
    const double* val;
    int n, nnz;
    int cs, ce;
    int ltile;
    int sys;
    int base;
    int span;
};
constexpr int kWinCap = 1408;
constexpr int kWinBufs = 2;
constexpr int kWinVecs = 2;

template <int kCap, int kStages, bool kPacked = false>
struct PipeGeom {
    static constexpr int kSlots = kCap + (kPacked ? 16 : 8);
    static constexpr int kEntryBytes = kPacked ? 6 : 12;
    static constexpr size_t kStageBytes = (size_t)kStages * kSlots * kEntryBytes;
    static constexpr size_t kWinBytes = (kPacked && kPackWindows) ? (size_t)kWinBufs * kWinVecs * kWinCap * 8 : 0;
    static constexpr size_t kBytes = kStageBytes + kWinBytes;
    static_assert(kStageBytes % 16 == 0, "windows start 16-byte aligned");
    static_assert(kCap % 8 == 0 && kCap >= 64, "stage capacity");
};
template <int kStages>
struct PipeBarriers {
    alignas(8) unsigned long long full[kStages];
    alignas(8) unsigned long long empty[kStages];
    alignas(8) unsigned long long wfull[kWinBufs];
    alignas(8) unsigned long long wempty[kWinBufs];
};
constexpr int kLsCap = 1536;
constexpr size_t kLsFusedBytes = 3 * ((size_t)(kLsCap + 8) * 12 + (kTileRows + 8) * 4 + kTileRows * 8) + 5 * kTileRows * 8;
constexpr size_t max3(size_t a, size_t b, size_t c) { return a > b ? (a > c ? a : c) : (b > c ? b : c); }
constexpr size_t kPipeRawBytes = max3(PipeGeom<kPipeCap, kPipeStages>::kBytes, PipeGeom<kPackCap, kPackStages, true>::kBytes, kLsFusedBytes);
struct PipeShared {
    alignas(16) unsigned char bytes[kPipeRawBytes];
    PipeBarriers<kMaxStages> bar;
};

template <bool kPacked = false>
__device__ __forceinline__ void tile_desc_fill(TileDesc& d, const CsrView& M, int ltile) {
    d.rowptr = M.rowptr;
    d.col = kPacked ? reinterpret_cast<const int*>(M.col16) : M.col;
    d.val = kPacked ? reinterpret_cast<const double*>(M.val32) : M.val;
    d.n = M.n;
    d.nnz = M.nnz;
    d.ltile = ltile;
    d.base = 0, d.span = 0;
    if (kPacked && M.rowptr) {
        const int2 info = __ldg(reinterpret_cast<const int2*>(M.tbase) + ltile);
        d.base = info.x;
        const int wlen = ((info.x + info.y + 1) & ~1) - (info.x & ~1);
        d.span = (info.y > 0 && wlen <= kWinCap) ? wlen : 0;
    }
    if (M.rowptr) {
        d.cs = __ldg(M.rowptr + min(ltile * kTileRows, M.n));
        d.ce = __ldg(M.rowptr + min((ltile + 1) * kTileRows, M.n));
    } else {
        d.cs = d.ce = 0;
    }
}

template <int kCap, int kStages, bool kPacked = false>
struct PipeT {
    static constexpr int kSlots = PipeGeom<kCap, kStages, kPacked>::kSlots;
    static constexpr bool kIsPacked = kPacked;
    using ValT = typename std::conditional<kPacked, float, double>::type;
    using ColT = typename std::conditional<kPacked, unsigned short, int>::type;
    static constexpr int kValUnit = 16 / (int)sizeof(ValT);
    static constexpr int kColUnit = 16 / (int)sizeof(ColT);
    static constexpr int kAlign = kColUnit > kValUnit ? kColUnit : kValUnit;
    ValT* val0;
    ColT* col0;
    unsigned long long* full;
    unsigned long long* empty;
    const TileDesc* tab;
    int ntiles;
    unsigned c_count;
    bool ghost;
    int role;
    unsigned p_count;
    int p_tile, p_blk;
    unsigned t_count;
    int flip;
    int early;
    int keep_l2;
#ifdef DPCG_PIPE_TRACE
    int tr_pos = 0;
    unsigned long long tr_phase = 0;
    __device__ __forceinline__ void tr_mark(unsigned long long label) {
        label += 8 * tr_phase;
        if (blockIdx.x == 0 && (threadIdx.x == 0 || threadIdx.x == 160) && tr_pos < kPipeTraceCap) {
            unsigned long long t;
            asm volatile("mov.u64 %0, %%globaltimer;" : "=l"(t));
            g_pipe_trace[threadIdx.x ? 1 : 0][tr_pos++] = (label << 48) | (t & 0xFFFFFFFFFFFFull);
        }
    }
#endif
    double* win0;
    unsigned long long* wfull;
    unsigned long long* wempty;
    unsigned w_issued, w_count;

    static __device__ __forceinline__ int blocks(const TileDesc& d) { return (d.ce - d.cs + kCap - 1) / kCap; }
    __device__ __forceinline__ const ValT* stage_val(unsigned s) const { return val0 + (size_t)s * kSlots; }
    __device__ __forceinline__ const ColT* stage_col(unsigned s) const { return col0 + (size_t)s * kSlots; }
    __device__ __forceinline__ void issue_copies(const TileDesc& d, unsigned stage, int as, int be, unsigned long long pol) {
        const unsigned ncol = (unsigned)(((be + kColUnit - 1) & ~(kColUnit - 1)) - as);
        const unsigned nval = (unsigned)(((be + kValUnit - 1) & ~(kValUnit - 1)) - as);
        unsigned long long* bar = &full[stage];
        mbar_arrive_expect_tx(bar, ncol * (unsigned)sizeof(ColT) + nval * (unsigned)sizeof(ValT));
        bulk_g2s(val0 + (size_t)stage * kSlots, reinterpret_cast<const ValT*>(d.val) + as, nval * (unsigned)sizeof(ValT), bar, pol);
        bulk_g2s(col0 + (size_t)stage * kSlots, reinterpret_cast<const ColT*>(d.col) + as, ncol * (unsigned)sizeof(ColT), bar, pol);
    }

    template <class Bars>
    __device__ __forceinline__ void init(unsigned char* bytes, Bars* bar, bool fresh = true) {
        val0 = reinterpret_cast<ValT*>(bytes);
        col0 = reinterpret_cast<ColT*>(bytes + (size_t)kStages * kSlots * sizeof(ValT));
        full = bar->full, empty = bar->empty;
        tab = nullptr;
        ntiles = 0;
        c_count = 0u, p_count = 0u, p_tile = 0, p_blk = 0, t_count = 0u, flip = 0, early = 0, keep_l2 = 0;
        ghost = threadIdx.x >= (unsigned)kBlock;
        role = threadIdx.x == (blockDim.x > (unsigned)kBlock ? (unsigned)kBlock : 0u) ? 0 : -1;
        win0 = reinterpret_cast<double*>(bytes + PipeGeom<kCap, kStages, kPacked>::kStageBytes);
        wfull = bar->wfull, wempty = bar->wempty;
        w_issued = 0u, w_count = 0u;
        if (fresh) {
            if (threadIdx.x == 0) {
#pragma unroll
                for (int s = 0; s < kStages; ++s) {
                    mbar_init(&full[s], 1u);
                    mbar_init(&empty[s], (unsigned)kWarpsPerBlock);
                }
                if (kPacked) {
#pragma unroll
                    for (int b = 0; b < kWinBufs; ++b) {
                        mbar_init(&wfull[b], 1u);
                        mbar_init(&wempty[b], (unsigned)kWarpsPerBlock);
                    }
                }
                mbar_fence_init();
            }
            __syncthreads();
        }
    }
    __device__ __forceinline__ void resume(unsigned items) { c_count = p_count = items; }

    __device__ __forceinline__ bool issue_one(bool blocking) {
        while (p_tile < ntiles) {
            if (p_blk < blocks(tab[p_tile])) break;
            ++p_tile, p_blk = 0;
        }
        if (p_tile >= ntiles) return false;
        if (p_count - c_count >= (unsigned)kStages) return false;
        const unsigned stage = p_count % kStages, use = p_count / kStages;
        if (use > 0) {
            const unsigned par = (use - 1u) & 1u;
            if (blocking) {
                while (!mbar_try_wait(&empty[stage], par)) {
                }
            } else if (!mbar_test_wait(&empty[stage], par)) {
                return false;
            }
        }
        const TileDesc& d = tab[p_tile];
        const int bs = d.cs + p_blk * kCap;
        const int be = min(d.ce, bs + kCap);
        const int as = bs & ~(kAlign - 1);
        issue_copies(d, stage, as, be, keep_l2 ? l2_policy_keep() : l2_policy_stream());
        DP_PIPE_MARK(7);
        ++p_blk, ++p_count;
        return true;
    }

    __device__ __forceinline__ void begin(const TileDesc* t, int count) {
        tab = t;
        ntiles = count;
        p_tile = 0, p_blk = 0;
        if (role >= 0) {
            while (issue_one(true)) {
            }
        }
    }

    __device__ __forceinline__ void issue_tile(int t) {
        const unsigned stage = p_count % kStages, use = p_count / kStages;
        if (use > 0) {
            while (!mbar_test_wait(&empty[stage], (use - 1u) & 1u)) {
            }
        }
        const TileDesc& d = tab[t];
        issue_copies(d, stage, d.cs & ~(kAlign - 1), d.ce, l2_policy_stream());
        ++p_count;
    }
    __device__ __forceinline__ unsigned wait_item() {
        const unsigned stage = c_count % kStages;
        while (!mbar_try_wait(&full[stage], (c_count / kStages) & 1u)) {
        }
        return stage;
    }

    __device__ __forceinline__ void begin_early(const TileDesc* t, int count, int id) {
        begin(t, count);
        early = id + 1;
    }
    __device__ __forceinline__ bool begin_resume(const TileDesc* t, int count, int id) {
        if (early != id + 1) return false;
        early = 0;
        tab = t, ntiles = count;
        return true;
    }
    __device__ __forceinline__ void drain_early() {
        if (!early) return;
        early = 0;
        int issued = 0;
        for (int t = 0; t < ntiles && issued < kStages; ++t) issued += blocks(tab[t]);
        issued = min(issued, kStages);
        if (role >= 0) p_tile = ntiles;
        for (int j = 0; j < issued; ++j) {
            const unsigned stage = c_count % kStages;
            while (!ghost && !mbar_try_wait(&full[stage], (c_count / kStages) & 1u)) {
            }
            release();
        }
    }

    __device__ __forceinline__ unsigned acquire() {
        if (role >= 0) {
            while (p_count <= c_count) issue_one(true);
            while (issue_one(false)) {
            }
        }
        DP_PIPE_MARK(6);
        const unsigned stage = c_count % kStages;
        const unsigned par = (c_count / kStages) & 1u;
        if (ghost) return stage;
#if DPCG_PIPE_WAIT_HINT
        while (!mbar_try_wait_hint(&full[stage], par, DPCG_PIPE_WAIT_HINT)) {
        }
#else
        while (!mbar_try_wait(&full[stage], par)) {
        }
#endif
        return stage;
    }
    __device__ __forceinline__ void release() {
        __syncwarp();
        if ((threadIdx.x & 31) == 0 && !ghost) mbar_arrive(&empty[c_count % kStages]);
        ++c_count;
    }

    static constexpr int kWinWarp = kWarpsPerBlock / 2;
    template <class Gather>
    __device__ __forceinline__ void window_issue(const TileDesc& t, const Gather& x) {
        if (blockDim.x > (unsigned)kBlock ? threadIdx.x == (unsigned)kBlock : threadIdx.x == kWinWarp * 32) {
            const unsigned buf = w_issued % kWinBufs, fill = w_issued / kWinBufs;
            if (fill > 0) {
                while (!mbar_try_wait_hint(&wempty[buf], (fill - 1u) & 1u, 1000u)) {
                }
            }
            const int off = t.base & ~1;
            const unsigned bytes = (unsigned)t.span * 8u;
            const unsigned long long pol = l2_policy_keep();
            asm volatile("fence.proxy.async;" ::: "memory");
            mbar_arrive_expect_tx(&wfull[buf], bytes * (unsigned)Gather::kVecs);
#pragma unroll
            for (int v = 0; v < Gather::kVecs; ++v)
                bulk_g2s(win0 + (size_t)(buf * kWinVecs + v) * kWinCap, x.vec(v) + off, bytes, &wfull[buf], pol);
        }
        ++w_issued;
    }
    template <class Gather>
    __device__ __forceinline__ const double* window_acquire(const TileDesc& d, const Gather& x) {
        if (w_issued == w_count) window_issue(d, x);
        const int next = (int)(&d - tab) + 1;
        if (next < ntiles && w_issued == w_count + 1u) {
            const TileDesc& nx = tab[next];
            if (nx.span > 0 && nx.sys == d.sys) window_issue(nx, x);
        }
        const unsigned buf = w_count % kWinBufs;
        while (!ghost && !mbar_try_wait_hint(&wfull[buf], (w_count / kWinBufs) & 1u, 1000u)) {
        }
        return win0 + (size_t)buf * kWinVecs * kWinCap;
    }
    __device__ __forceinline__ void window_release() {
        __syncwarp();
        if ((threadIdx.x & 31) == 0 && !ghost) mbar_arrive(&wempty[w_count % kWinBufs]);
        ++w_count;
    }

    template <int kUnroll, class Load>
    __device__ __forceinline__ double consume_items(const TileDesc& d, int rs, int re, bool compute, const Load& load) {
        double sum = 0.0;
        const int nb = blocks(d);
        for (int j = 0; j < nb; ++j) {
            const int bs = d.cs + j * kCap;
            const int be = min(d.ce, bs + kCap);
            const int as = bs & ~(kAlign - 1);
            const unsigned stage = acquire();
            DP_PIPE_MARK(2);
            if (compute && !ghost) {
                const ValT* __restrict__ sv = stage_val(stage);
                const ColT* __restrict__ sc = stage_col(stage);
                const int qe = min(re, be) - as;
                for (int q = max(rs, bs) - as; q < qe; q += kUnroll) {
                    int c[kUnroll];
                    double v[kUnroll], xv[kUnroll];
#pragma unroll
                    for (int u = 0; u < kUnroll; ++u) {
                        const bool on = q + u < qe;
                        c[u] = on ? (int)sc[q + u] : 0;
                        v[u] = on ? (double)sv[q + u] : 0.0;
                    }
#pragma unroll
                    for (int u = 0; u < kUnroll; ++u) xv[u] = (q + u < qe) ? load(c[u]) : 0.0;
#pragma unroll
                    for (int u = 0; u < kUnroll; ++u)
                        if (q + u < qe) sum = __dadd_rn(sum, __dmul_rn(v[u], xv[u]));
                }
            }
            DP_PIPE_MARK(3);
            release();
        }
        return sum;
    }

    template <int kUnroll = kPipeUnroll, class Gather>
    __device__ __forceinline__ double tile_spmv(const TileDesc& d, int rs, int re, const Gather& x, bool compute) {
        if constexpr (kPacked && kPackWindows && Gather::kVecs > 0) {
            if (d.span > 0) {
                DP_PIPE_MARK(0);
                const double* w = window_acquire(d, x);
                DP_PIPE_MARK(1);
                const int shift = d.base & 1;
                const double sum = consume_items<kUnroll>(d, rs, re, compute, [&](int c16) {
                    return x.combine(w[c16 + shift], Gather::kVecs > 1 ? w[kWinCap + c16 + shift] : 0.0);
                });
                window_release();
                DP_PIPE_MARK(4);
                return sum;
            }
        }
        const int base = kPacked ? d.base : 0;
        DP_PIPE_MARK(0);
        const double sum = consume_items<kUnroll>(d, rs, re, compute, [&](int c) { return x(base + c); });
        DP_PIPE_MARK(4);
        return sum;
    }

    __device__ __forceinline__ void tile_skip(const TileDesc& d) {
        if (kPacked && kPackWindows && d.span > 0 && w_issued > w_count) {
            const unsigned buf = w_count % kWinBufs;
            while (!ghost && !mbar_try_wait(&wfull[buf], (w_count / kWinBufs) & 1u)) {
            }
            window_release();
        }
        consume_items<1>(d, 0, 0, false, [](int) { return 0.0; });
    }
};

using Pipe = PipeT<kPipeCap, kPipeStages>;
using PipePacked = PipeT<kPackCap, kPackStages, true>;

__device__ __forceinline__ void tile_row_extent(const TileDesc& d, int& rs, int& re) {
    rs = re = 0;
    if (d.rowptr) {
        const int row = d.ltile * kTileRows + (int)threadIdx.x;
        rs = __ldg(d.rowptr + min(row, d.n));
        re = __ldg(d.rowptr + min(row + 1, d.n));
    }
}

constexpr int kReduceSlots = 3 * kWarpsPerBlock;

template <int kN, class P>
__device__ __forceinline__ void tile_reduce(double (&v)[kN], double (*scratch2x)[kReduceSlots], P& pipe) {
    static_assert(kN <= 3, "scratch holds 3 values per warp");
    const int lane = threadIdx.x & 31, warp = threadIdx.x >> 5;
    double* scratch = scratch2x[pipe.flip];
    pipe.flip ^= 1;
#pragma unroll
    for (int i = 0; i < kN; ++i) v[i] = warp_sum(v[i]);
    if (lane == 0 && warp < kWarpsPerBlock) {
#pragma unroll
        for (int i = 0; i < kN; ++i) scratch[i * kWarpsPerBlock + warp] = v[i];
    }
    __syncthreads();
#pragma unroll
    for (int i = 0; i < kN; ++i) v[i] = half_warp_sum(scratch[i * kWarpsPerBlock + (lane & (kWarpsPerBlock - 1))]);
}


constexpr int kRedRing = 8;
static_assert(kMaxStages < kRedRing, "reduction ring must outlast the warps' maximum distance");

struct TileRed {
    double slot[kRedRing][3][kWarpsPerBlock];
    int count[kRedRing];
};

template <int kN, class P, class Write>
__device__ __forceinline__ void tile_reduce_async(double (&v)[kN], TileRed& red, P& pipe, const Write& write) {
    static_assert(kN <= 3, "ring slots hold 3 values per warp");
    const int lane = threadIdx.x & 31, warp = threadIdx.x >> 5;
    const unsigned r = pipe.t_count % kRedRing;
    ++pipe.t_count;
    if (pipe.ghost) return;
#pragma unroll
    for (int i = 0; i < kN; ++i) v[i] = warp_sum(v[i]);
    int old = 0;
    if (lane == 0) {
#pragma unroll
        for (int i = 0; i < kN; ++i) red.slot[r][i][warp] = v[i];
        __threadfence_block();
        old = atomicAdd(&red.count[r], 1);
    }
    old = __shfl_sync(kFull, old, 0);
    if (old == kWarpsPerBlock - 1) {
        __threadfence_block();
#pragma unroll
        for (int i = 0; i < kN; ++i) v[i] = half_warp_sum(red.slot[r][i][lane & (kWarpsPerBlock - 1)]);
        if (lane == 0) {
            red.count[r] = 0;
            write(v);
        }
    }
}

}
```

deeppreconditioning_b200/sparse.py:

```python

from __future__ import annotations

import numpy as np
import torch

from . import _lib

_MODES = {"tril": _lib.ASSEMBLE_TRIL, "tril_t": _lib.ASSEMBLE_TRIL_T, "symmetrise": _lib.ASSEMBLE_SYMMETRISE}


def _cuda_device(device=None) -> torch.device:
    if device is None:
        device = torch.device("cuda", torch.cuda.current_device())
    device = torch.device(device)
    if device.type != "cuda":
        raise _lib.DpcgError("deeppreconditioning_b200 runs on CUDA devices only (no CPU fallback)")
    return device


def _workspace(nbytes: int, device) -> torch.Tensor:
    return torch.empty(max(int(nbytes), 256), dtype=torch.uint8, device=device)


class CsrMatrix:

    def __init__(self, rowptr: torch.Tensor, col: torch.Tensor, val: torch.Tensor, n: int) -> None:
        assert rowptr.dtype == torch.int32 and col.dtype == torch.int32 and val.dtype == torch.float64
        assert rowptr.is_cuda and col.is_cuda and val.is_cuda
        self.rowptr, self.col, self.val, self.n = rowptr.contiguous(), col.contiguous(), val.contiguous(), int(n)
        self._t: CsrMatrix | None = None
        self._dinv: torch.Tensor | None = None
        self._packed = None
        self._packed_key = None

    @classmethod
    def from_spconv(cls, tensor, original_size: int, mode: str = "tril", batch: int = 0) -> "CsrMatrix":
        n = int(original_size)
        indices, features = tensor.indices, tensor.features
        device = _cuda_device(indices.device if indices.is_cuda else None)
        indices = indices.to(device=device, dtype=torch.int32).contiguous()
        feats = features.detach().to(device=device, dtype=torch.float32)
        feats = (feats[:, 0] if feats.dim() == 2 else feats).contiguous()
        nnz_in = int(indices.shape[0])
        cap = max(nnz_in * (2 if mode == "symmetrise" else 1), 1)
        rowptr = torch.empty(n + 1, dtype=torch.int32, device=device)
        col = torch.empty(cap, dtype=torch.int32, device=device)
        val = torch.empty(cap, dtype=torch.float64, device=device)
        nnz_out = torch.zeros(1, dtype=torch.int32, device=device)
        flag = torch.zeros(1, dtype=torch.int32, device=device)
        lib = _lib.lib()
        ws = _workspace(lib.dp_csr_from_coo_workspace_bytes(n, nnz_in), device)
        with torch.cuda.device(device):
            _lib.check(lib.dp_csr_from_coo(_lib.ptr(indices), _lib.ptr(feats), nnz_in, int(batch), n, _MODES[mode],
                                           _lib.ptr(rowptr), _lib.ptr(col), _lib.ptr(val), _lib.ptr(nnz_out),
                                           _lib.ptr(flag), _lib.ptr(ws), ws.numel(), _lib.stream_ptr(device)),
                       "dp_csr_from_coo")
        nnz = int(nnz_out.item())
        _lib.raise_on_flag(flag, "dp_csr_from_coo (duplicate (row, col) in the COO input)")
        col, val = col[:nnz], val[:nnz]
        if cap > nnz + nnz // 4:
            col, val = col.clone(), val.clone()
        return cls(rowptr, col, val, n)

    @classmethod
    def from_arrays(cls, rowptr, col, val, device=None) -> "CsrMatrix":
        device = _cuda_device(device)
        def as_t(a, dt):
            t = torch.as_tensor(np.asarray(a) if not torch.is_tensor(a) else a)
            return t.to(device=device, dtype=dt, non_blocking=bool(t.device.type == "cpu" and t.is_pinned() and t.dtype == dt))
        rowptr = as_t(rowptr, torch.int32)
        return cls(rowptr, as_t(col, torch.int32), as_t(val, torch.float64), rowptr.shape[0] - 1)

    @classmethod
    def from_torch(cls, matrix: torch.Tensor, device=None) -> "CsrMatrix":
        if device is None and matrix.is_cuda:
            device = matrix.device
        if matrix.layout == torch.strided:
            matrix = matrix.to_sparse_csr()
        elif matrix.layout != torch.sparse_csr:
            matrix = matrix.coalesce().to_sparse_csr() if matrix.layout == torch.sparse_coo else matrix.to_sparse_csr()
        return cls.from_arrays(matrix.crow_indices(), matrix.col_indices(), matrix.values(), device)

    @classmethod
    def from_scipy(cls, matrix, device=None) -> "CsrMatrix":
        m = matrix.tocsr()
        m.sort_indices()
        return cls.from_arrays(m.indptr, m.indices, m.data, device)

    @property
    def shape(self):
        return (self.n, self.n)

    @property
    def nnz(self) -> int:
        return int(self.col.shape[0])

    @property
    def device(self):
        return self.val.device

    def values(self) -> torch.Tensor:
        return self.val

    def transpose(self) -> "CsrMatrix":
        if self._t is None:
            n, nnz, dev = self.n, self.nnz, self.device
            rowptr = torch.empty(n + 1, dtype=torch.int32, device=dev)
            col = torch.empty(max(nnz, 1), dtype=torch.int32, device=dev)
            val = torch.empty(max(nnz, 1), dtype=torch.float64, device=dev)
            lib = _lib.lib()
            ws = _workspace(lib.dp_csr_transpose_workspace_bytes(n, nnz), dev)
            with torch.cuda.device(dev):
                _lib.check(lib.dp_csr_transpose(n, nnz, _lib.ptr(self.rowptr), _lib.ptr(self.col), _lib.ptr(self.val),
                                                _lib.ptr(rowptr), _lib.ptr(col), _lib.ptr(val), _lib.ptr(ws),
                                                ws.numel(), _lib.stream_ptr(dev)), "dp_csr_transpose")
            self._t = CsrMatrix(rowptr, col[:nnz], val[:nnz], n)
            self._t._t = self
        return self._t

    @property
    def T(self) -> "CsrMatrix":
        return self.transpose()

    def tril(self) -> "CsrMatrix":
        counts = torch.diff(self.rowptr).long()
        rows = torch.repeat_interleave(torch.arange(self.n, device=self.device), counts)
        keep = self.col.long() <= rows
        per_row = torch.bincount(rows[keep], minlength=self.n)
        rowptr = torch.zeros(self.n + 1, dtype=torch.int32, device=self.device)
        rowptr[1:] = torch.cumsum(per_row, 0).to(torch.int32)
        return CsrMatrix(rowptr, self.col[keep].contiguous(), self.val[keep].contiguous(), self.n)

    def packed(self) -> "PackedCsr | None":
        pack_many([self])
        return self._packed or None

    def matvec(self, x: torch.Tensor, out: torch.Tensor | None = None, packed: bool = False) -> torch.Tensor:
        assert x.is_cuda and x.dtype == torch.float64 and x.shape == (self.n,)
        x = x.contiguous()
        y = out if out is not None else torch.empty(self.n, dtype=torch.float64, device=self.device)
        if packed:
            pk = self.packed()
            if pk is None:
                raise _lib.DpcgError("matrix has no exact packed copy (values beyond fp32 or a tile wider than 65535 columns)")
            with torch.cuda.device(self.device):
                _lib.check(_lib.lib().dp_spmv_csr_packed_f64(self.n, self.nnz, _lib.ptr(self.rowptr), _lib.ptr(pk.col16),
                                                             _lib.ptr(pk.val32), _lib.ptr(pk.tile_base), _lib.ptr(x),
                                                             _lib.ptr(y), _lib.stream_ptr(self.device)),
                           "dp_spmv_csr_packed_f64")
            return y
        with torch.cuda.device(self.device):
            _lib.check(_lib.lib().dp_spmv_csr_f64(self.n, self.nnz, _lib.ptr(self.rowptr), _lib.ptr(self.col),
                                                  _lib.ptr(self.val), _lib.ptr(x), _lib.ptr(y),
                                                  _lib.stream_ptr(self.device)), "dp_spmv_csr_f64")
        return y

    def __matmul__(self, x: torch.Tensor) -> torch.Tensor:
        y = self.matvec(x.to(device=self.device, dtype=torch.float64))
        return y if x.is_cuda else y.to(x.device)

    def inv_diagonal(self) -> torch.Tensor:
        if self._dinv is None:
            dinv = torch.empty(self.n, dtype=torch.float64, device=self.device)
            flag = torch.zeros(1, dtype=torch.int32, device=self.device)
            with torch.cuda.device(self.device):
                _lib.check(_lib.lib().dp_csr_inv_diagonal(self.n, _lib.ptr(self.rowptr), _lib.ptr(self.col),
                                                          _lib.ptr(self.val), _lib.ptr(dinv), _lib.ptr(flag),
                                                          _lib.stream_ptr(self.device)), "dp_csr_inv_diagonal")
            _lib.raise_on_flag(flag, "dp_csr_inv_diagonal (row without a stored diagonal)")
            self._dinv = dinv
        return self._dinv

    def to_host(self):
        return self.rowptr.cpu().numpy(), self.col.cpu().numpy(), self.val.cpu().numpy()

    def to_torch_csr(self, device="cpu") -> torch.Tensor:
        return torch.sparse_csr_tensor(self.rowptr.to(device).long(), self.col.to(device).long(), self.val.to(device),
                                       size=self.shape)


class PackedCsr:

    def __init__(self, col16: torch.Tensor, val32: torch.Tensor, tile_base: torch.Tensor) -> None:
        self.col16, self.val32, self.tile_base = col16, val32, tile_base


def pack_many(matrices) -> None:
    todo, seen = [], set()
    for m in matrices:
        key = (m.col._version, m.val._version, m.col.data_ptr(), m.val.data_ptr())
        if id(m) in seen or (m._packed is not None and m._packed_key == key):
            continue
        seen.add(id(m))
        m._packed, m._packed_key = None, key
        todo.append(m)
    if not todo:
        return
    lib = _lib.lib()
    tile_rows = int(lib.dp_csr_pack_tile_rows())
    by_device = {}
    for m in todo:
        by_device.setdefault(m.device, []).append(m)
    for dev, ms in by_device.items():
        status = torch.zeros(len(ms), dtype=torch.int32, device=dev)
        copies = []
        with torch.cuda.device(dev):
            for i, m in enumerate(ms):
                nnz = m.nnz
                col16 = torch.empty(max((nnz + 7) // 8 * 8, 8), dtype=torch.uint16, device=dev)
                val32 = torch.empty(max((nnz + 3) // 4 * 4, 4), dtype=torch.float32, device=dev)
                tile_base = torch.empty((max((m.n + tile_rows - 1) // tile_rows, 1), 2), dtype=torch.int32, device=dev)
                _lib.check(lib.dp_csr_pack(m.n, nnz, _lib.ptr(m.rowptr), _lib.ptr(m.col), _lib.ptr(m.val), _lib.ptr(col16),
                                           _lib.ptr(val32), _lib.ptr(tile_base), status.data_ptr() + 4 * i,
                                           _lib.stream_ptr(dev)), "dp_csr_pack")
                copies.append(PackedCsr(col16, val32, tile_base))
        verdicts = status.cpu().tolist()
        for m, pk, bad in zip(ms, copies, verdicts):
            m._packed = pk if bad == 0 else False


def as_csr(matrix, device=None) -> CsrMatrix:
    if isinstance(matrix, CsrMatrix):
        return matrix
    if torch.is_tensor(matrix):
        return CsrMatrix.from_torch(matrix, device)
    if hasattr(matrix, "tocsr"):
        return CsrMatrix.from_scipy(matrix, device)
    raise TypeError(f"cannot interpret {type(matrix).__name__} as a sparse matrix")
```

include/dpcg.h:

```cpp
#ifndef DPCG_H
#define DPCG_H

#include <stddef.h>
#include <stdint.h>

#ifdef __cplusplus
extern "C" {
#endif

#define DP_VERSION 100

enum dp_status {
    DP_OK = 0,
    DP_ERR_INVALID = 1,
    DP_ERR_ALIGNMENT = 2,
    DP_ERR_WORKSPACE = 3,
    DP_ERR_CUDA = 4,
    DP_ERR_STRUCTURE = 5,
    DP_ERR_TIMEOUT = 6
};

enum dp_precond {
    DP_PRECOND_IDENTITY = 0,
    DP_PRECOND_JACOBI = 1,
    DP_PRECOND_MULTIPLY = 2,
    DP_PRECOND_SOLVE = 3,
    DP_PRECOND_CSR = 4
};

enum dp_engine {
    DP_ENGINE_FUSED = 0,
    DP_ENGINE_STEPPED = 1
};

enum dp_assemble_mode {
    DP_ASSEMBLE_TRIL = 0,
    DP_ASSEMBLE_TRIL_T = 1,
    DP_ASSEMBLE_SYMMETRISE = 2
};

int dp_version(void);
const char* dp_status_string(int status);
const char* dp_last_cuda_error(void);
int dp_device_info(int* sm_count_host, int* pcg_ctas_per_sm_host, int* l2_bytes_host);

size_t dp_csr_from_coo_workspace_bytes(int32_t n, int64_t nnz_in);
int dp_csr_from_coo(const int32_t* indices, const float* features, int64_t nnz_in, int32_t batch, int32_t n,
                    int32_t mode, int32_t* rowptr, int32_t* col, double* val, int32_t* nnz_out, int32_t* flag_out,
                    void* workspace, size_t workspace_bytes, void* stream);

size_t dp_csr_transpose_workspace_bytes(int32_t n, int32_t nnz);
int dp_csr_transpose(int32_t n, int32_t nnz, const int32_t* rowptr, const int32_t* col, const double* val,
                     int32_t* rowptr_t, int32_t* col_t, double* val_t, void* workspace, size_t workspace_bytes,
                     void* stream);

int dp_csr_inv_diagonal(int32_t n, const int32_t* rowptr, const int32_t* col, const double* val, double* dinv,
                        int32_t* flag_out, void* stream);

int dp_csr_aat_nnz(int32_t n, const int32_t* rowptr, const int32_t* col, const int32_t* rowptr_t, const int32_t* col_t,
                   int64_t* nnz_out, void* stream);

int32_t dp_csr_pack_tile_rows(void);
int dp_csr_pack(int32_t n, int32_t nnz, const int32_t* rowptr, const int32_t* col, const double* val, uint16_t* col16,
                float* val32, int32_t* tile_base, int32_t* status_out, void* stream);
int dp_spmv_csr_packed_f64(int32_t n, int32_t nnz, const int32_t* rowptr, const uint16_t* col16, const float* val32,
                           const int32_t* tile_base, const double* x, double* y, void* stream);

int dp_spmv_csr_f64(int32_t n, int32_t nnz, const int32_t* rowptr, const int32_t* col, const double* val,
                    const double* x, double* y, void* stream);

int dp_coo_spmv_batch_f32(const int32_t* indices, const float* features, int64_t nnz, int32_t nbatch, int32_t n,
                          const float* vec, int32_t transpose, float* out, void* stream);

size_t dp_sptrsv_analyse_workspace_bytes(int32_t n);
int dp_sptrsv_analyse(int32_t n, const int32_t* rowptr, const int32_t* col, int32_t upper, int32_t* level,
                      int32_t* perm, int32_t* level_ptr, int32_t* nlevels_out, int32_t* flag_out, void* workspace,
                      size_t workspace_bytes, void* stream);

int64_t dp_sptrsv_plan_chunks(int32_t nlevels, const int32_t* level_ptr_host);
size_t dp_sptrsv_plan_sizes_workspace_bytes(int32_t n);
int dp_sptrsv_plan_sizes(int32_t n, const int32_t* nlevels, const int32_t* level_ptr, int32_t* chunk_ptr,
                         int32_t* summary_out, void* workspace, size_t workspace_bytes, void* stream);
int dp_sptrsv_plan_build(int32_t n, int32_t nlevels, const int32_t* perm, const int32_t* level_ptr,
                         const int32_t* chunk_ptr, int32_t* plan, int64_t nchunks, void* stream);

size_t dp_sptrsv_permute_workspace_bytes(int32_t n);
int dp_sptrsv_permute(int32_t n, int32_t upper, const int32_t* rowptr, const int32_t* col, const double* val, const int32_t* perm,
                      const int32_t* level, int32_t* rowptr_p, int32_t* col_p, double* val_p, int32_t* level_sorted,
                      int32_t* stats_out, void* workspace, size_t workspace_bytes, void* stream);

size_t dp_sptrsv_workspace_bytes(void);
int dp_sptrsv_solve_f64(int32_t n, const int32_t* rowptr, const int32_t* col, const double* val, int32_t upper,
                        const int32_t* plan, int64_t nchunks, int32_t max_level_chunks, const double* b, double* x,
                        int32_t* flag_out, void* workspace, size_t workspace_bytes, void* stream);

typedef struct dp_trsv_system {
    int32_t n;
    int32_t upper;
    int32_t max_level_chunks;
    int32_t reserved;
    int64_t nchunks;
    const int32_t* rowptr; const int32_t* col; const double* val;
    const int32_t* plan;
    const double* b;
    double* x;
} dp_trsv_system_t;
size_t dp_sptrsv_batch_workspace_bytes(int32_t nsys);
int dp_sptrsv_solve_batch_f64(const dp_trsv_system_t* systems_host, int32_t nsys, int32_t* flag_out, void* workspace,
                              size_t workspace_bytes, void* stream);

typedef struct dp_trsv_ls_system {
    int32_t n;
    int32_t nnz;
    int32_t upper;
    int32_t flags;
    const int32_t* rowptr_p; const int32_t* col_p; const double* val_p;
    const int32_t* perm;
    const int32_t* level_sorted;
    const double* b;
    double* x;
} dp_trsv_ls_system_t;
void dp_sptrsv_ls_limits(int32_t* limits_host );
size_t dp_sptrsv_ls_workspace_bytes(int32_t nsys);
int dp_sptrsv_ls_solve_batch_f64(const dp_trsv_ls_system_t* systems_host, int32_t nsys, void* workspace,
                                 size_t workspace_bytes, void* stream);
int dp_sptrsv_ls_prepare(const dp_trsv_ls_system_t* systems_host, int32_t nsys, void* workspace, size_t workspace_bytes,
                         void* stream);
int dp_sptrsv_ls_launch(int32_t nsys, void* workspace, size_t workspace_bytes, void* stream);

#define DP_TRSV_REVERSED 1
#define DP_TRSV_SHORT_ROWS 2
void dp_sptrsv_ts_limits(int32_t* limits_host );
size_t dp_sptrsv_ts_workspace_bytes(const dp_trsv_ls_system_t* systems_host, int32_t nsys);
int dp_sptrsv_ts_solve_batch_f64(const dp_trsv_ls_system_t* systems_host, int32_t nsys, int32_t* flag_out, void* workspace,
                                 size_t workspace_bytes, void* stream);
int dp_sptrsv_ts_prepare(const dp_trsv_ls_system_t* systems_host, int32_t nsys, void* workspace, size_t workspace_bytes,
                         void* stream);
int dp_sptrsv_ts_launch(int32_t nsys, int32_t max_tiles, int32_t nmax, int32_t short_rows, int32_t nperm, int32_t* flag_out,
                        void* workspace, void* stream);

int dp_ic0_f64(int32_t n, const int32_t* rowptr, const int32_t* col, const double* a_val, double* l_val,
               const int32_t* plan, int64_t nchunks, int32_t max_level_chunks, int32_t* flag_out, void* workspace,
               size_t workspace_bytes, void* stream);

int dp_icholt_host(int32_t n, const int32_t* rowptr_host, const int32_t* col_host, const double* val_host, int32_t fill_in,
                   double threshold, int32_t* rowptr_out_host, int32_t* col_out_host, double* val_out_host,
                   int64_t capacity, int64_t* nnz_out_host);

typedef struct dp_pcg_system {
    int32_t n;
    int32_t precond;
    int32_t a_nnz, m_nnz, mt_nnz;
    int32_t fwd_nchunks, bwd_nchunks;
    int32_t fwd_max_level_chunks, bwd_max_level_chunks;
    int32_t solve_algorithm;
    const int32_t* a_rowptr; const int32_t* a_col; const double* a_val;
    const int32_t* m_rowptr; const int32_t* m_col; const double* m_val;
    const int32_t* mt_rowptr; const int32_t* mt_col; const double* mt_val;
    const double* dinv;
    const int32_t* fwd_plan; const int32_t* bwd_plan;
    const int32_t* fwd_ls_rowptr; const int32_t* fwd_ls_col; const double* fwd_ls_val;
    const int32_t* fwd_ls_perm; const int32_t* fwd_ls_level;
    const int32_t* bwd_ls_rowptr; const int32_t* bwd_ls_col; const double* bwd_ls_val;
    const int32_t* bwd_ls_perm; const int32_t* bwd_ls_level;
    const double* b;
    double* x;
    double* work;
    int32_t* iters_out;
    double* res_out;
    double* history;
    double* coef;
    const uint16_t* a_col16; const float* a_val32; const int32_t* a_tile_base;
    const uint16_t* m_col16; const float* m_val32; const int32_t* m_tile_base;
    const uint16_t* mt_col16; const float* mt_val32; const int32_t* mt_tile_base;
} dp_pcg_system_t;

#define DP_SOLVE_TILE_STREAM 1
#define DP_SOLVE_SHORT_ROWS 2

typedef struct dp_pcg_params {
    double rtol;
    int32_t max_iter;
    int32_t engine;
    int32_t check_every;
    int32_t reserved;
} dp_pcg_params_t;

int64_t dp_pcg_work_doubles(int32_t n);
size_t dp_pcg_workspace_bytes(int32_t nsys);
int dp_pcg_solve_f64(const dp_pcg_system_t* systems_host, int32_t nsys, const dp_pcg_params_t* params_host,
                     int32_t* flag_out, void* workspace, size_t workspace_bytes, void* stream);

size_t dp_spconv_sort_workspace_bytes(int32_t batch_size, int32_t h);
int dp_spconv_sort_sites(const int32_t* indices, int64_t nnz, int32_t batch_size, int32_t h, int32_t w, int32_t* rowptr,
                         int32_t* col, int32_t* perm, int32_t* flag_out, void* workspace, size_t workspace_bytes,
                         void* stream);
size_t dp_spconv_rules_workspace_bytes(int32_t batch_size, int32_t h, int32_t ph);
int dp_spconv_rules_count(const int32_t* rowptr_in, const int32_t* col_in, int32_t batch_size, int32_t h, int32_t w,
                          int32_t ph, int32_t pw, int32_t* rowptr_out, void* workspace, size_t workspace_bytes,
                          void* stream);
int dp_spconv_rules_fill(const int32_t* rowptr_in, const int32_t* col_in, const int32_t* perm, int32_t batch_size,
                         int32_t h, int32_t w, int32_t ph, int32_t pw, const int32_t* rowptr_out, int32_t* col_out,
                         int32_t* rules, int32_t* indices_out, void* stream);
typedef struct dp_spconv_layer {
    int64_t nout;
    int32_t ntaps;
    int32_t cin, cout;
    int32_t reserved;
    const int32_t* src;
    const float* in;
    const float* weight;
    const float* bias;
    const float* slope;
    const float* head_weight;
    const float* head_bias;
    const int32_t* indices;
    float* out;
} dp_spconv_layer_t;
int dp_spconv_layer_f32(const dp_spconv_layer_t* layer_host, void* stream);

int dp_debug_pcg_trace(const void* workspace, int32_t nsys, int64_t* out_host, int32_t capacity);
int dp_debug_pipe_trace(uint64_t* out_host, int32_t capacity, int32_t unit );

#ifdef __cplusplus
}
#endif
#endif
```

Measured before the change: 19.12.

## Add DIA stream format for banded matrices in fused PCG kernel

Adds a diagonal (DIA) storage format holding float32 values per tile and diagonal, built on device from CSR when a matrix has at most 16 diagonals. The fused PCG kernel gains a DIA pipeline variant that streams only the values and computes column indices from the diagonal offsets, so no column index arrays are read. It is selected by default whenever packing is enabled and every matrix converts. The aim is to cut SpMV memory traffic and gather irregularity. The cost is padding for diagonals that are partly empty and an extra conversion step.

```diff
diff --git a/deeppreconditioning_b200/_lib.py b/deeppreconditioning_b200/_lib.py
--- a/deeppreconditioning_b200/_lib.py
+++ b/deeppreconditioning_b200/_lib.py
@@ -16,6 +16,9 @@
 PRECOND_IDENTITY, PRECOND_JACOBI, PRECOND_MULTIPLY, PRECOND_SOLVE, PRECOND_CSR = range(5)
 ENGINE_FUSED, ENGINE_STEPPED = 0, 1
 ASSEMBLE_TRIL, ASSEMBLE_TRIL_T, ASSEMBLE_SYMMETRISE = 0, 1, 2
+STREAM_FORMATS = ("f64", "packed", "dia")
+DIA_MAX_DIAGONALS = 16
+DIA_META = 2 + 2 * DIA_MAX_DIAGONALS
 
 _p = C.c_void_p
 _i32 = C.c_int32
@@ -34,6 +37,16 @@
             "b", "x", "work", "iters_out", "res_out", "history", "coef",
             "a_col16", "a_val32", "a_tile_base", "m_col16", "m_val32", "m_tile_base",
             "mt_col16", "mt_val32", "mt_tile_base")]
+
+
+class DiaCopy(C.Structure):
+
+    _fields_ = [("val", _p), ("ndiag", _i32), ("off", _i32 * DIA_MAX_DIAGONALS), ("reserved", _i32)]
+
+
+class PcgDia(C.Structure):
+
+    _fields_ = [("a", DiaCopy), ("m", DiaCopy), ("mt", DiaCopy)]
 
 
 class TrsvSystem(C.Structure):
@@ -78,6 +91,7 @@
     "dp_csr_pack_tile_rows": (_i32, []),
     "dp_csr_pack": (C.c_int, [_i32, _i32, _p, _p, _p, _p, _p, _p, _p, _p]),
     "dp_spmv_csr_packed_f64": (C.c_int, [_i32, _i32, _p, _p, _p, _p, _p, _p, _p]),
+    "dp_csr_dia": (C.c_int, [_i32, _i32, _p, _p, _p, _p, _i64, _p, _p]),
     "dp_coo_spmv_batch_f32": (C.c_int, [_p, _p, _i64, _i32, _i32, _p, _i32, _p, _p]),
     "dp_sptrsv_analyse_workspace_bytes": (C.c_size_t, [_i32]),
     "dp_sptrsv_analyse": (C.c_int, [_i32, _p, _p, _i32, _p, _p, _p, _p, _p, _p, C.c_size_t, _p]),
@@ -114,6 +128,9 @@
     "dp_debug_pcg_trace": (C.c_int, [_p, _i32, _p, _i32]),
     "dp_debug_pipe_trace": (C.c_int, [_p, _i32, _i32]),
     "dp_pcg_solve_f64": (C.c_int, [C.POINTER(PcgSystem), _i32, C.POINTER(PcgParams), _p, _p, C.c_size_t, _p]),
+    "dp_pcg_solve_dia_f64": (C.c_int, [C.POINTER(PcgSystem), C.POINTER(PcgDia), _i32, C.POINTER(PcgParams), _p, _p,
+                                       C.c_size_t, _p]),
+    "dp_pcg_stream_format": (C.c_int, [C.POINTER(PcgSystem), C.POINTER(PcgDia), _i32, C.POINTER(PcgParams)]),
 }
 
 EXPORTED_SYMBOLS = tuple(_SIGNATURES)
diff --git a/deeppreconditioning_b200/cg.py b/deeppreconditioning_b200/cg.py
--- a/deeppreconditioning_b200/cg.py
+++ b/deeppreconditioning_b200/cg.py
@@ -32,6 +32,14 @@
         return kappa_estimate(self.alphas, self.betas) if self.alphas else float("nan")
 
 
+def fill_dia(copy: _lib.DiaCopy, matrix: CsrMatrix) -> None:
+    dc = matrix._dia or None
+    copy.val = _lib.ptr(dc.val) if dc is not None else None
+    copy.ndiag = dc.ndiag if dc is not None else 0
+    for k, o in enumerate(dc.offsets if dc is not None else []):
+        copy.off[k] = o
+
+
 def stopping_criterion(_, rk, b):
     return torch.inner(rk, rk) / torch.inner(b, b)
 
@@ -39,7 +47,8 @@
 class PcgBatch:
 
     def __init__(self, systems, rtol: float = 1e-8, max_iter: int = 1024, engine: str = "fused",
-                 check_every: int = 32, history: bool = False, device=None, pack: bool = True) -> None:
+                 check_every: int = 32, history: bool = False, device=None, pack: bool = True, dia: bool | None = None) -> None:
+        dia = pack if dia is None else bool(dia)
         if not systems:
             raise ValueError("empty batch")
         self.device = torch.device(device) if device is not None else None
@@ -70,13 +79,14 @@
         if any(getattr(e["M"], "tile_stream", False) for e in self.entries):
             self.params = _lib.PcgParams(self.rtol, self.max_iter, _ENGINES["stepped"], min(int(check_every), 8), 0)
         solve_mode = any(e["M"].precond == _lib.PRECOND_SOLVE for e in self.entries)
-        if pack and engine == "fused" and not solve_mode:
-            pack_many([m for e in self.entries for m in [e["A"], *e["M"].stream_matrices()]])
+        if (pack or dia) and engine == "fused" and not solve_mode:
+            pack_many([m for e in self.entries for m in [e["A"], *e["M"].stream_matrices()]], pack=pack, dia=dia)
         self.iters = torch.full((nsys,), -1, dtype=torch.int32, device=self.device)
         self.res = torch.full((nsys,), float("nan"), dtype=torch.float64, device=self.device)
         self.flag = torch.zeros(1, dtype=torch.int32, device=self.device)
         self.ws = _workspace(lib.dp_pcg_workspace_bytes(nsys), self.device)
         self.descs = (_lib.PcgSystem * nsys)()
+        self.dia_descs = (_lib.PcgDia * nsys)()
         for i, e in enumerate(self.entries):
             d, A = self.descs[i], e["A"]
             d.n, d.a_nnz = A.n, A.nnz
@@ -92,6 +102,12 @@
             d.res_out = self.res.data_ptr() + 8 * i
             d.history = _lib.ptr(e["hist"])
             d.coef = _lib.ptr(e["coef"])
+            if dia:
+                for tag, m in zip(("a", "m", "mt"), [A, *e["M"].stream_matrices()]):
+                    fill_dia(getattr(self.dia_descs[i], tag), m)
+        fmt = _lib.lib().dp_pcg_stream_format(self.descs, self.dia_descs, nsys, ctypes.byref(self.params))
+        _lib.check(-fmt if fmt < 0 else 0, "dp_pcg_stream_format")
+        self.stream_format = _lib.STREAM_FORMATS[fmt]
 
     def __len__(self) -> int:
         return len(self.entries)
@@ -107,9 +123,9 @@
 
     def solve(self) -> None:
         with torch.cuda.device(self.device):
-            _lib.check(_lib.lib().dp_pcg_solve_f64(self.descs, len(self.entries), ctypes.byref(self.params),
-                                                   _lib.ptr(self.flag), _lib.ptr(self.ws), self.ws.numel(),
-                                                   _lib.stream_ptr(self.device)), "dp_pcg_solve_f64")
+            _lib.check(_lib.lib().dp_pcg_solve_dia_f64(self.descs, self.dia_descs, len(self.entries),
+                                                       ctypes.byref(self.params), _lib.ptr(self.flag), _lib.ptr(self.ws),
+                                                       self.ws.numel(), _lib.stream_ptr(self.device)), "dp_pcg_solve_dia_f64")
 
     def results(self, seconds: float = 0.0) -> list[PcgResult]:
         _lib.raise_on_flag(self.flag, "dp_pcg_solve_f64")
@@ -136,8 +152,8 @@
 
 
 def pcg_solve_batch(systems, rtol: float = 1e-8, max_iter: int = 1024, engine: str = "fused", check_every: int = 32,
-                    history: bool = False, device=None, pack: bool = True) -> list[PcgResult]:
-    batch = PcgBatch(systems, rtol, max_iter, engine, check_every, history, device, pack)
+                    history: bool = False, device=None, pack: bool = True, dia: bool | None = None) -> list[PcgResult]:
+    batch = PcgBatch(systems, rtol, max_iter, engine, check_every, history, device, pack, dia)
     torch.cuda.synchronize(batch.device)
     start = time.perf_counter()
     batch.solve()
@@ -146,8 +162,8 @@
 
 
 def pcg_solve(A, b, M=None, x0=None, rtol: float = 1e-8, max_iter: int = 1024, engine: str = "fused",
-              check_every: int = 32, history: bool = False, pack: bool = True) -> PcgResult:
-    return pcg_solve_batch([(A, b, M, x0)], rtol, max_iter, engine, check_every, history, pack=pack)[0]
+              check_every: int = 32, history: bool = False, pack: bool = True, dia: bool | None = None) -> PcgResult:
+    return pcg_solve_batch([(A, b, M, x0)], rtol, max_iter, engine, check_every, history, pack=pack, dia=dia)[0]
 
 
 def preconditioned_conjugate_gradient(A, b: torch.Tensor, M, x0=None, x_true=None, rtol=1e-8, max_iter=1024):
diff --git a/deeppreconditioning_b200/csrc/pcg.cu b/deeppreconditioning_b200/csrc/pcg.cu
--- a/deeppreconditioning_b200/csrc/pcg.cu
+++ b/deeppreconditioning_b200/csrc/pcg.cu
@@ -37,6 +37,7 @@
     double* res_out;
     double* history;
     double* coef;
+    dp_dia_t A_dia, M_dia, Mt_dia;
 };
 
 struct Ctx {
@@ -451,7 +452,14 @@
     if (kPhase == PH_DOTRZ) phase_dotrz<kInit>(ctx, S, d, k, sm, sc, pipe);
 }
 
-template <int kTab, bool kPacked>
+template <int kTab>
+__device__ __forceinline__ const dp_dia_t* dia_of(const SysDev& S) {
+    if (kTab == TAB_A) return &S.A_dia;
+    if (kTab == TAB_P1) return S.precond == DP_PRECOND_MULTIPLY ? &S.Mt_dia : &S.M_dia;
+    return S.precond == DP_PRECOND_MULTIPLY ? &S.M_dia : nullptr;
+}
+
+template <int kTab, int kFmt>
 __device__ __forceinline__ void build_table(const Ctx& ctx, int cur, int ga, int gb, Smem& sm) {
     const int count = __ldcg(ctx.act_meta + 2 * cur);
     const int* asys = ctx.act_sys[cur];
@@ -463,23 +471,28 @@
         const int lt = g - __ldcg(aofs + seg);
         const SysDev* S = ctx.sys + s;
         const int precond = S->precond;
-        CsrView M{nullptr, nullptr, nullptr, 0, 0};
-        if (kTab == TAB_A) M = S->A;
-        if (kTab == TAB_P1 && precond == DP_PRECOND_MULTIPLY) M = S->Mt;
-        if (kTab == TAB_P1 && precond == DP_PRECOND_CSR) M = S->M;
-        if (kTab == TAB_P2 && precond == DP_PRECOND_MULTIPLY) M = S->M;
         TileDesc d;
-        tile_desc_fill<kPacked>(d, M, lt);
+        if constexpr (kFmt == kFmtDia) {
+            const dp_dia_t* V = dia_of<kTab>(*S);
+            tile_desc_fill_dia(d, V ? V->val : nullptr, V ? V->ndiag : 0, V ? V->off : nullptr, S->n, lt);
+        } else {
+            CsrView M{nullptr, nullptr, nullptr, 0, 0};
+            if (kTab == TAB_A) M = S->A;
+            if (kTab == TAB_P1 && precond == DP_PRECOND_MULTIPLY) M = S->Mt;
+            if (kTab == TAB_P1 && precond == DP_PRECOND_CSR) M = S->M;
+            if (kTab == TAB_P2 && precond == DP_PRECOND_MULTIPLY) M = S->M;
+            tile_desc_fill<kFmt == kFmtPacked>(d, M, lt);
+        }
         d.sys = s;
         sm.tab[kTab][i] = d;
     }
 }
 
-template <int kTab, bool kPacked>
+template <int kTab, int kFmt>
 __device__ __forceinline__ void ensure_table(const Ctx& ctx, int cur, int ver, int ga, int gb, Smem& sm) {
     if (sm.tab_ver[kTab] == ver && sm.tab_ga[kTab] == ga && sm.tab_gb[kTab] == gb) return;
     __syncthreads();
-    build_table<kTab, kPacked>(ctx, cur, ga, gb, sm);
+    build_table<kTab, kFmt>(ctx, cur, ga, gb, sm);
     if (threadIdx.x == 0) sm.tab_ver[kTab] = ver, sm.tab_ga[kTab] = ga, sm.tab_gb[kTab] = gb;
     __syncthreads();
 }
@@ -497,7 +510,7 @@
 #endif
     for (int ga = g0; ga < g1; ga += kMaxRoundTiles) {
         const int gb = min(g1, ga + kMaxRoundTiles);
-        ensure_table<kTab, P::kIsPacked>(ctx, cur, ver, ga, gb, sm);
+        ensure_table<kTab, P::kFormat>(ctx, cur, ver, ga, gb, sm);
         const TileDesc* tab = sm.tab[kTab];
         if (kStream) {
             if (!pipe.begin_resume(tab, gb - ga, kTab)) {
@@ -508,6 +521,10 @@
         for (int i = 0; i < gb - ga; ++i) {
             const TileDesc& d = tab[i];
             const SysDev& S = load_sys(ctx, d.sys, sm);
+            if constexpr (P::kDia) {
+                const dp_dia_t* V = dia_of<kTab>(S);
+                pipe.dia_off = V ? smem_u32(V->off) : 0u;
+            }
             int rs = 0, re = 0;
             if (kStream) tile_row_extent(d, rs, re);
             run_tile<kPhase, kInit, kCheckState>(ctx, S, d, rs, re, k, sm, sc, pipe);
@@ -595,10 +612,10 @@
 }
 
 constexpr int kFusedThreadsPacked = kPackProducerWarp ? kBlock + kWarp : kBlock;
-template <bool kSolve, bool kPacked>
-__global__ void __launch_bounds__(kPacked ? kFusedThreadsPacked : kBlock, 2) pcg_fused_kernel(Ctx ctx) {
+template <bool kSolve, int kFmt>
+__global__ void __launch_bounds__(kFmt != kFmtF64 ? kFusedThreadsPacked : kBlock, 2) pcg_fused_kernel(Ctx ctx) {
     extern __shared__ __align__(16) unsigned char smem_raw[];
-    typename std::conditional<kPacked, PipePacked, Pipe>::type pipe;
+    typename std::conditional<kFmt == kFmtDia, PipeDia, typename std::conditional<kFmt == kFmtPacked, PipePacked, Pipe>::type>::type pipe;
     Smem& sm = smem_init(smem_raw, pipe);
     pipe.keep_l2 = ctx.keep_l2;
     GridBarrier bar{ctx.word, ctx.flag, &sm.bcast, 0u, gridDim.x};
@@ -856,6 +873,31 @@
     return DP_OK;
 }
 
+static bool dia_given(const dp_dia_t& V) {
+    return V.val && aligned16(V.val) && V.ndiag >= 0 && V.ndiag <= kDiaMax;
+}
+static int stream_format(const dp_pcg_system_t* systems, const dp_pcg_dia_t* dia, int nsys, const dp_pcg_params_t& params) {
+    if (params.engine != DP_ENGINE_FUSED) return DP_STREAM_F64;
+    bool packed = true, diag = dia != nullptr;
+    auto has_pack = [](const uint16_t* col16, const float* val32, const int32_t* tbase) {
+        return col16 && val32 && tbase && aligned16(col16) && aligned16(val32);
+    };
+    for (int i = 0; i < nsys; ++i) {
+        const dp_pcg_system_t& u = systems[i];
+        if (u.precond == DP_PRECOND_SOLVE) return DP_STREAM_F64;
+        const bool m = u.precond == DP_PRECOND_MULTIPLY || u.precond == DP_PRECOND_CSR, mt = u.precond == DP_PRECOND_MULTIPLY;
+        if (!has_pack(u.a_col16, u.a_val32, u.a_tile_base) || (m && !has_pack(u.m_col16, u.m_val32, u.m_tile_base)) ||
+            (mt && !has_pack(u.mt_col16, u.mt_val32, u.mt_tile_base)))
+            packed = false;
+        if (diag && (!dia_given(dia[i].a) || (m && !dia_given(dia[i].m)) || (mt && !dia_given(dia[i].mt)))) diag = false;
+    }
+    const char* e = getenv("DPCG_NO_PACK");
+    if (e && e[0] == '1') packed = false;
+    e = getenv("DPCG_NO_DIA");
+    if (e && e[0] == '1') diag = false;
+    return diag ? DP_STREAM_DIA : packed ? DP_STREAM_PACKED : DP_STREAM_F64;
+}
+
 }
 
 using namespace dp;
@@ -877,8 +919,8 @@
     if (sm_count_host) *sm_count_host = sms;
     if (l2_bytes_host) *l2_bytes_host = l2;
     if (pcg_ctas_per_sm_host) {
-        if (allow_smem(pcg_fused_kernel<false, false>) != DP_OK) return DP_ERR_CUDA;
-        *pcg_ctas_per_sm_host = coop_grid((const void*)pcg_fused_kernel<false, false>, kBlock, sizeof(Smem)) / (sms > 0 ? sms : 1);
+        if (allow_smem(pcg_fused_kernel<false, kFmtF64>) != DP_OK) return DP_ERR_CUDA;
+        *pcg_ctas_per_sm_host = coop_grid((const void*)pcg_fused_kernel<false, kFmtF64>, kBlock, sizeof(Smem)) / (sms > 0 ? sms : 1);
     }
     return DP_OK;
 }
@@ -907,8 +949,20 @@
 #endif
 }
 
+int dp_pcg_stream_format(const dp_pcg_system_t* systems_host, const dp_pcg_dia_t* dia_host, int32_t nsys,
+                         const dp_pcg_params_t* params_host) {
+    if (!systems_host || nsys <= 0 || !params_host) return -DP_ERR_INVALID;
+    return stream_format(systems_host, dia_host, nsys, *params_host);
+}
+
 int dp_pcg_solve_f64(const dp_pcg_system_t* systems_host, int32_t nsys, const dp_pcg_params_t* params_host,
                      int32_t* flag_out, void* workspace, size_t workspace_bytes, void* stream) {
+    return dp_pcg_solve_dia_f64(systems_host, nullptr, nsys, params_host, flag_out, workspace, workspace_bytes, stream);
+}
+
+int dp_pcg_solve_dia_f64(const dp_pcg_system_t* systems_host, const dp_pcg_dia_t* dia_host, int32_t nsys,
+                         const dp_pcg_params_t* params_host, int32_t* flag_out, void* workspace, size_t workspace_bytes,
+                         void* stream) {
     if (!systems_host || nsys <= 0 || !params_host || !flag_out || !workspace) return DP_ERR_INVALID;
     if (params_host->max_iter < 0) return DP_ERR_INVALID;
     if (!aligned16(workspace)) return DP_ERR_ALIGNMENT;
@@ -921,8 +975,8 @@
     std::vector<int> tile_ofs((size_t)nsys + 1, 0), fwd_ofs((size_t)nsys + 1, 0), bwd_ofs((size_t)nsys + 1, 0);
     std::vector<int> ident((size_t)nsys + 1, 0);
     int has_multiply = 0, has_solve = 0, has_ls = 0, n_solve = 0, n_ts = 0;
-    bool packed = true;
-    long long working_set_bytes = 0, matrix_entries = 0;
+    const int format = stream_format(systems_host, dia_host, nsys, *params_host);
+    long long working_set_bytes = 0, matrix_entries = 0, dia_bytes = 0;
     long long sum_fwd_lvl = 0, sum_bwd_lvl = 0;
     std::vector<TsSysDev> ts_sys[4];
     std::vector<int> ts_owner;
@@ -939,12 +993,13 @@
         d.A = CsrView{u.a_rowptr, u.a_col, u.a_val, u.n, u.a_nnz, u.a_col16, u.a_val32, u.a_tile_base};
         d.M = CsrView{u.m_rowptr, u.m_col, u.m_val, u.n, u.m_nnz, u.m_col16, u.m_val32, u.m_tile_base};
         d.Mt = CsrView{u.mt_rowptr, u.mt_col, u.mt_val, u.n, u.mt_nnz, u.mt_col16, u.mt_val32, u.mt_tile_base};
-        {
-            auto has_pack = [](const CsrView& V) { return V.col16 && V.val32 && V.tbase && aligned16(V.col16) && aligned16(V.val32); };
-            if (!has_pack(d.A)) packed = false;
-            if ((u.precond == DP_PRECOND_MULTIPLY || u.precond == DP_PRECOND_CSR) && !has_pack(d.M)) packed = false;
-            if (u.precond == DP_PRECOND_MULTIPLY && !has_pack(d.Mt)) packed = false;
-            if (u.precond == DP_PRECOND_SOLVE) packed = false;
+        if (format == DP_STREAM_DIA) {
+            const dp_pcg_dia_t& v = dia_host[i];
+            auto bytes = [&](const dp_dia_t& V) { return 4ll * V.ndiag * kTileRows * ntiles_of(u.n); };
+            d.A_dia = v.a;
+            dia_bytes += bytes(v.a);
+            if (u.precond == DP_PRECOND_MULTIPLY || u.precond == DP_PRECOND_CSR) d.M_dia = v.m, dia_bytes += bytes(v.m);
+            if (u.precond == DP_PRECOND_MULTIPLY) d.Mt_dia = v.mt, dia_bytes += bytes(v.mt);
         }
         d.dinv = u.dinv;
         d.fwd_plan = u.fwd_plan;
@@ -1042,15 +1097,12 @@
     }
 
     if (n_ts && (n_ts != n_solve || params_host->engine != DP_ENGINE_STEPPED)) return DP_ERR_INVALID;
-    {
-        const char* e = getenv("DPCG_NO_PACK");
-        if ((e && e[0] == '1') || params_host->engine != DP_ENGINE_FUSED) packed = false;
-    }
-    const void* fused = has_solve ? (const void*)pcg_fused_kernel<true, false>
-                        : packed  ? (const void*)pcg_fused_kernel<false, true>
-                                  : (const void*)pcg_fused_kernel<false, false>;
+    const void* fused = has_solve                    ? (const void*)pcg_fused_kernel<true, kFmtF64>
+                        : format == DP_STREAM_DIA    ? (const void*)pcg_fused_kernel<false, kFmtDia>
+                        : format == DP_STREAM_PACKED ? (const void*)pcg_fused_kernel<false, kFmtPacked>
+                                                     : (const void*)pcg_fused_kernel<false, kFmtF64>;
     if (allow_dynamic_smem(fused, sizeof(Smem)) != DP_OK || allow_smem(pcg_phase_kernel<PH_FWD, false>) != DP_OK) return DP_ERR_CUDA;
-    const int fused_threads = (!has_solve && packed) ? kFusedThreadsPacked : kBlock;
+    const int fused_threads = (!has_solve && format != DP_STREAM_F64) ? kFusedThreadsPacked : kBlock;
     const int coop = coop_grid(fused, fused_threads, sizeof(Smem));
     const int coop_phase = coop_grid((const void*)pcg_phase_kernel<PH_FWD, false>, kBlock, sizeof(Smem));
     auto clamp_pw = [](long long lvl_chunks, int grid) {
@@ -1083,7 +1135,8 @@
         DP_CUDA(cudaGetDevice(&dev));
         DP_CUDA(cudaDeviceGetAttribute(&l2, cudaDevAttrL2CacheSize, dev));
         const char* e = getenv("DPCG_KEEP_L2");
-        if (packed) working_set_bytes -= matrix_entries * 6;
+        if (format == DP_STREAM_PACKED) working_set_bytes -= matrix_entries * 6;
+        if (format == DP_STREAM_DIA) working_set_bytes += dia_bytes - matrix_entries * 12;
         ctx.keep_l2 = e ? (e[0] == '1') : (working_set_bytes * 10 < (long long)l2 * 6);
     }
     ctx.rtol = params_host->rtol;
diff --git a/deeppreconditioning_b200/csrc/spmv.cu b/deeppreconditioning_b200/csrc/spmv.cu
--- a/deeppreconditioning_b200/csrc/spmv.cu
+++ b/deeppreconditioning_b200/csrc/spmv.cu
@@ -96,6 +96,96 @@
     if (bad) atomicOr(status, bad);
 }
 
+constexpr int kDiaEmpty = (int)0x80000000;
+
+__global__ void dia_init_kernel(int* __restrict__ meta) {
+    const int i = threadIdx.x;
+    if (i < 2 + kDiaMax) meta[i] = 0;
+    else if (i < DP_DIA_META) meta[i] = kDiaEmpty;
+}
+
+__device__ __forceinline__ bool dia_set_insert(int* tab, int v) {
+    for (int i = 0; i < kDiaMax; ++i) {
+        int t = *(volatile int*)(tab + i);
+        if (t == v) return true;
+        if (t == kDiaEmpty) {
+            t = atomicCAS(tab + i, kDiaEmpty, v);
+            if (t == kDiaEmpty || t == v) return true;
+        }
+    }
+    return false;
+}
+
+__global__ void __launch_bounds__(kBlock)
+dia_scan_kernel(int n, const int* __restrict__ rowptr, const int* __restrict__ col, const double* __restrict__ val,
+                int* __restrict__ meta) {
+    __shared__ int tab[kDiaMax];
+    __shared__ int bad_s;
+    if (threadIdx.x < kDiaMax) tab[threadIdx.x] = kDiaEmpty;
+    if (threadIdx.x == 0) bad_s = 0;
+    __syncthreads();
+    const int row = blockIdx.x * kTileRows + (int)threadIdx.x;
+    int bad = 0;
+    if (row < n) {
+        const int rs = __ldg(rowptr + row), re = __ldg(rowptr + row + 1);
+        int prev = -1;
+        for (int q = rs; q < re; ++q) {
+            const int c = __ldg(col + q);
+            const double v = __ldg(val + q);
+            if (c <= prev) bad |= 4;
+            prev = c;
+            if (as_bits((double)(float)v) != as_bits(v)) bad |= 1;
+            if (!dia_set_insert(tab, c - row)) bad |= 2;
+        }
+    }
+    if (bad) atomicOr(&bad_s, bad);
+    __syncthreads();
+    if (threadIdx.x < kDiaMax && tab[threadIdx.x] != kDiaEmpty && !dia_set_insert(meta + 2 + kDiaMax, tab[threadIdx.x]))
+        atomicOr(meta, 2);
+    if (threadIdx.x == 0 && bad_s) atomicOr(meta, bad_s);
+}
+
+__global__ void __launch_bounds__(kBlock)
+dia_fill_kernel(int n, int nnz, const int* __restrict__ rowptr, const int* __restrict__ col, const double* __restrict__ val,
+                float* __restrict__ out, long long capacity, int* __restrict__ meta) {
+    __shared__ int off[kDiaMax];
+    __shared__ int nd_s;
+    if (threadIdx.x < kDiaMax) {
+        const int* set = meta + 2 + kDiaMax;
+        const int v = __ldcg(set + threadIdx.x);
+        int rank = 0, count = 0;
+        for (int j = 0; j < kDiaMax; ++j) {
+            const int w = __ldcg(set + j);
+            if (w != kDiaEmpty) ++count, rank += w < v;
+        }
+        if (v != kDiaEmpty) off[rank] = v;
+        if (threadIdx.x == 0) nd_s = count;
+    }
+    __syncthreads();
+    const int nd = nd_s;
+    const long long ntiles = ((long long)n + kTileRows - 1) / kTileRows;
+    int status = __ldcg(meta);
+    if (!(status & 2)) {
+        if (4ll * nnz < 3ll * nd * n) status |= 8;
+        else if (ntiles * nd * kTileRows > capacity) status |= 16;
+    }
+    if (blockIdx.x == 0 && threadIdx.x == 0) {
+        meta[0] = status;
+        meta[1] = nd;
+        for (int d = 0; d < nd; ++d) meta[2 + d] = off[d];
+    }
+    if (status) return;
+    const int row = blockIdx.x * kTileRows + (int)threadIdx.x;
+    int q = 0, re = 0;
+    if (row < n) q = __ldg(rowptr + row), re = __ldg(rowptr + row + 1);
+    float* dst = out + (size_t)blockIdx.x * nd * kTileRows + threadIdx.x;
+    for (int d = 0; d < nd; ++d) {
+        float v = 0.0f;
+        if (q < re && __ldg(col + q) - row == off[d]) v = (float)__ldg(val + q), ++q;
+        dst[(size_t)d * kTileRows] = v;
+    }
+}
+
 __global__ void coo_spmv_batch_kernel(const int* __restrict__ ind, const float* __restrict__ feat, long long nnz,
                                       int nbatch, int n, const float* __restrict__ vec, int transpose,
                                       float* __restrict__ out) {
@@ -235,6 +325,23 @@
     return DP_OK;
 }
 
+int dp_csr_dia(int32_t n, int32_t nnz, const int32_t* rowptr, const int32_t* col, const double* val, float* val_out,
+               int64_t capacity, int32_t* meta_out, void* stream) {
+    if (n < 0 || nnz < 0 || capacity < 0 || !rowptr || !meta_out || (n > 0 && !val_out) || (nnz > 0 && (!col || !val)))
+        return DP_ERR_INVALID;
+    if (!aligned16(val_out)) return DP_ERR_ALIGNMENT;
+    cudaStream_t s = (cudaStream_t)stream;
+    dia_init_kernel<<<1, DP_DIA_META, 0, s>>>(meta_out);
+    DP_LAUNCH_CHECK();
+    if (n == 0) return DP_OK;
+    const int tiles = (n + kTileRows - 1) / kTileRows;
+    dia_scan_kernel<<<tiles, kBlock, 0, s>>>(n, rowptr, col, val, meta_out);
+    DP_LAUNCH_CHECK();
+    dia_fill_kernel<<<tiles, kBlock, 0, s>>>(n, nnz, rowptr, col, val, val_out, capacity, meta_out);
+    DP_LAUNCH_CHECK();
+    return DP_OK;
+}
+
 int dp_spmv_csr_packed_f64(int32_t n, int32_t nnz, const int32_t* rowptr, const uint16_t* col16, const float* val32,
                            const int32_t* tile_base, const double* x, double* y, void* stream) {
     if (n < 0 || nnz < 0 || !rowptr || !y || !tile_base || (nnz > 0 && (!col16 || !val32 || !x))) return DP_ERR_INVALID;
diff --git a/deeppreconditioning_b200/csrc/tilepipe.cuh b/deeppreconditioning_b200/csrc/tilepipe.cuh
--- a/deeppreconditioning_b200/csrc/tilepipe.cuh
+++ b/deeppreconditioning_b200/csrc/tilepipe.cuh
@@ -60,7 +60,17 @@
 constexpr int kPackStages = DPCG_PACK_STAGES;
 constexpr bool kPackWindows = DPCG_PACK_WINDOWS != 0;
 constexpr bool kPackProducerWarp = DPCG_PACK_PRODUCER_WARP != 0;
-constexpr int kMaxStages = kPipeStages > kPackStages ? kPipeStages : kPackStages;
+#ifndef DPCG_DIA_STAGES
+#define DPCG_DIA_STAGES 2
+#endif
+
+enum StreamFmt { kFmtF64 = 0, kFmtPacked = 1, kFmtDia = 2 };
+constexpr int kDiaMax = DP_DIA_MAX_DIAGONALS;
+constexpr int kDiaCap = kDiaMax * kTileRows;
+constexpr int kDiaStages = DPCG_DIA_STAGES;
+constexpr int kMaxStages = (kPipeStages > kPackStages ? kPipeStages : kPackStages) > kDiaStages
+                               ? (kPipeStages > kPackStages ? kPipeStages : kPackStages)
+                               : kDiaStages;
 
 __device__ __forceinline__ unsigned smem_u32(const void* p) { return (unsigned)__cvta_generic_to_shared(p); }
 __device__ __forceinline__ void mbar_init(unsigned long long* bar, unsigned count) {
@@ -179,10 +189,11 @@
 constexpr int kWinBufs = 2;
 constexpr int kWinVecs = 2;
 
-template <int kCap, int kStages, bool kPacked = false>
+template <int kCap, int kStages, int kFmt = kFmtF64>
 struct PipeGeom {
-    static constexpr int kSlots = kCap + (kPacked ? 16 : 8);
-    static constexpr int kEntryBytes = kPacked ? 6 : 12;
+    static constexpr bool kPacked = kFmt == kFmtPacked;
+    static constexpr int kSlots = kFmt == kFmtDia ? kCap : kCap + (kPacked ? 16 : 8);
+    static constexpr int kEntryBytes = kFmt == kFmtDia ? 4 : kPacked ? 6 : 12;
     static constexpr size_t kStageBytes = (size_t)kStages * kSlots * kEntryBytes;
     static constexpr size_t kWinBytes = (kPacked && kPackWindows) ? (size_t)kWinBufs * kWinVecs * kWinCap * 8 : 0;
     static constexpr size_t kBytes = kStageBytes + kWinBytes;
@@ -199,7 +210,9 @@
 constexpr int kLsCap = 1536;
 constexpr size_t kLsFusedBytes = 3 * ((size_t)(kLsCap + 8) * 12 + (kTileRows + 8) * 4 + kTileRows * 8) + 5 * kTileRows * 8;
 constexpr size_t max3(size_t a, size_t b, size_t c) { return a > b ? (a > c ? a : c) : (b > c ? b : c); }
-constexpr size_t kPipeRawBytes = max3(PipeGeom<kPipeCap, kPipeStages>::kBytes, PipeGeom<kPackCap, kPackStages, true>::kBytes, kLsFusedBytes);
+constexpr size_t kPipeRawBytes = max3(max3(PipeGeom<kPipeCap, kPipeStages>::kBytes, PipeGeom<kPackCap, kPackStages, kFmtPacked>::kBytes,
+                                           PipeGeom<kDiaCap, kDiaStages, kFmtDia>::kBytes),
+                                      kLsFusedBytes, 0);
 struct PipeShared {
     alignas(16) unsigned char bytes[kPipeRawBytes];
     PipeBarriers<kMaxStages> bar;
@@ -228,11 +241,42 @@
     }
 }
 
-template <int kCap, int kStages, bool kPacked = false>
-struct PipeT {
-    static constexpr int kSlots = PipeGeom<kCap, kStages, kPacked>::kSlots;
-    static constexpr bool kIsPacked = kPacked;
-    using ValT = typename std::conditional<kPacked, float, double>::type;
+__device__ __forceinline__ void tile_desc_fill_dia(TileDesc& d, const float* val, int ndiag, const int* off, int n, int ltile) {
+    const int nd = val ? ndiag : 0;
+    d.rowptr = nullptr;
+    d.col = nullptr;
+    d.val = reinterpret_cast<const double*>(val + (size_t)ltile * nd * kTileRows);
+    d.n = n;
+    d.nnz = 0;
+    d.cs = 0, d.ce = nd;
+    d.ltile = ltile;
+    d.base = 0, d.span = 0;
+    if (nd > 0) {
+        const int b = ltile * kTileRows;
+        const int lo = max(0, b + off[0]), hi = min(n, b + kTileRows + off[nd - 1]);
+        if (hi > lo) d.base = lo, d.span = hi - lo;
+    }
+}
+
+template <bool kDia>
+struct DiaState {};
+template <>
+struct DiaState<true> {
+    unsigned dia_off;
+    __device__ __forceinline__ int off(int k) const {
+        int v;
+        asm volatile("ld.shared.s32 %0, [%1];" : "=r"(v) : "r"(dia_off + 4u * (unsigned)k));
+        return v;
+    }
+};
+
+template <int kCap, int kStages, int kFmt = kFmtF64>
+struct PipeT : DiaState<kFmt == kFmtDia> {
+    static constexpr int kSlots = PipeGeom<kCap, kStages, kFmt>::kSlots;
+    static constexpr int kFormat = kFmt;
+    static constexpr bool kPacked = kFmt == kFmtPacked;
+    static constexpr bool kDia = kFmt == kFmtDia;
+    using ValT = typename std::conditional<kFmt != kFmtF64, float, double>::type;
     using ColT = typename std::conditional<kPacked, unsigned short, int>::type;
     static constexpr int kValUnit = 16 / (int)sizeof(ValT);
     static constexpr int kColUnit = 16 / (int)sizeof(ColT);
@@ -269,7 +313,10 @@
     unsigned long long* wempty;
     unsigned w_issued, w_count;
 
-    static __device__ __forceinline__ int blocks(const TileDesc& d) { return (d.ce - d.cs + kCap - 1) / kCap; }
+    static __device__ __forceinline__ int blocks(const TileDesc& d) {
+        if constexpr (kDia) return d.ce > d.cs ? 1 : 0;
+        return (d.ce - d.cs + kCap - 1) / kCap;
+    }
     __device__ __forceinline__ const ValT* stage_val(unsigned s) const { return val0 + (size_t)s * kSlots; }
     __device__ __forceinline__ const ColT* stage_col(unsigned s) const { return col0 + (size_t)s * kSlots; }
     __device__ __forceinline__ void issue_copies(const TileDesc& d, unsigned stage, int as, int be, unsigned long long pol) {
@@ -291,7 +338,7 @@
         c_count = 0u, p_count = 0u, p_tile = 0, p_blk = 0, t_count = 0u, flip = 0, early = 0, keep_l2 = 0;
         ghost = threadIdx.x >= (unsigned)kBlock;
         role = threadIdx.x == (blockDim.x > (unsigned)kBlock ? (unsigned)kBlock : 0u) ? 0 : -1;
-        win0 = reinterpret_cast<double*>(bytes + PipeGeom<kCap, kStages, kPacked>::kStageBytes);
+        win0 = reinterpret_cast<double*>(bytes + PipeGeom<kCap, kStages, kFmt>::kStageBytes);
         wfull = bar->wfull, wempty = bar->wempty;
         w_issued = 0u, w_count = 0u;
         if (fresh) {
@@ -333,10 +380,17 @@
             }
         }
         const TileDesc& d = tab[p_tile];
-        const int bs = d.cs + p_blk * kCap;
-        const int be = min(d.ce, bs + kCap);
-        const int as = bs & ~(kAlign - 1);
-        issue_copies(d, stage, as, be, keep_l2 ? l2_policy_keep() : l2_policy_stream());
+        const unsigned long long pol = keep_l2 ? l2_policy_keep() : l2_policy_stream();
+        if constexpr (kDia) {
+            const unsigned bytes = (unsigned)(d.ce * kTileRows) * 4u;
+            mbar_arrive_expect_tx(&full[stage], bytes);
+            bulk_g2s(val0 + (size_t)stage * kSlots, d.val, bytes, &full[stage], pol);
+        } else {
+            const int bs = d.cs + p_blk * kCap;
+            const int be = min(d.ce, bs + kCap);
+            const int as = bs & ~(kAlign - 1);
+            issue_copies(d, stage, as, be, pol);
+        }
         DP_PIPE_MARK(7);
         ++p_blk, ++p_count;
         return true;
@@ -494,8 +548,42 @@
         return sum;
     }
 
+    template <int kUnroll, class Gather>
+    __device__ __forceinline__ double dia_tile(const TileDesc& d, const Gather& x, bool compute) {
+        double sum = 0.0;
+        if (d.ce <= d.cs) return sum;
+        const int nd = d.ce;
+        const int row = d.ltile * kTileRows + (int)threadIdx.x;
+        const int last = d.n - 1;
+        const bool work = compute && !ghost;
+        const unsigned stage = acquire();
+        DP_PIPE_MARK(2);
+        if (work) {
+            const float* __restrict__ sv = stage_val(stage) + threadIdx.x;
+#pragma unroll 1
+            for (int d0 = 0; d0 < nd; d0 += kUnroll) {
+                double xv[kUnroll];
+#pragma unroll
+                for (int u = 0; u < kUnroll; ++u)
+                    xv[u] = d0 + u < nd ? x(min(max(row + this->off(d0 + u), 0), last)) : 0.0;
+#pragma unroll
+                for (int u = 0; u < kUnroll; ++u)
+                    if (d0 + u < nd) sum = __dadd_rn(sum, __dmul_rn((double)sv[(d0 + u) * kTileRows], xv[u]));
+            }
+        }
+        DP_PIPE_MARK(3);
+        release();
+        return sum;
+    }
+
     template <int kUnroll = kPipeUnroll, class Gather>
     __device__ __forceinline__ double tile_spmv(const TileDesc& d, int rs, int re, const Gather& x, bool compute) {
+        if constexpr (kDia) {
+            DP_PIPE_MARK(0);
+            const double sum = dia_tile<kUnroll>(d, x, compute);
+            DP_PIPE_MARK(4);
+            return sum;
+        }
         if constexpr (kPacked && kPackWindows && Gather::kVecs > 0) {
             if (d.span > 0) {
                 DP_PIPE_MARK(0);
@@ -529,7 +617,8 @@
 };
 
 using Pipe = PipeT<kPipeCap, kPipeStages>;
-using PipePacked = PipeT<kPackCap, kPackStages, true>;
+using PipePacked = PipeT<kPackCap, kPackStages, kFmtPacked>;
+using PipeDia = PipeT<kDiaCap, kDiaStages, kFmtDia>;
 
 __device__ __forceinline__ void tile_row_extent(const TileDesc& d, int& rs, int& re) {
     rs = re = 0;
diff --git a/deeppreconditioning_b200/sparse.py b/deeppreconditioning_b200/sparse.py
--- a/deeppreconditioning_b200/sparse.py
+++ b/deeppreconditioning_b200/sparse.py
@@ -32,6 +32,8 @@
         self._dinv: torch.Tensor | None = None
         self._packed = None
         self._packed_key = None
+        self._dia = None
+        self._dia_key = None
 
     @classmethod
     def from_spconv(cls, tensor, original_size: int, mode: str = "tril", batch: int = 0) -> "CsrMatrix":
@@ -135,6 +137,10 @@
         pack_many([self])
         return self._packed or None
 
+    def dia(self) -> "DiaCsr | None":
+        pack_many([self], pack=False, dia=True)
+        return self._dia or None
+
     def matvec(self, x: torch.Tensor, out: torch.Tensor | None = None, packed: bool = False) -> torch.Tensor:
         assert x.is_cuda and x.dtype == torch.float64 and x.shape == (self.n,)
         x = x.contiguous()
@@ -185,26 +191,56 @@
         self.col16, self.val32, self.tile_base = col16, val32, tile_base
 
 
-def pack_many(matrices) -> None:
-    todo, seen = [], set()
+class DiaCsr:
+
+    def __init__(self, val: torch.Tensor, offsets: list) -> None:
+        self.val, self.offsets = val, list(offsets)
+
+    @property
+    def ndiag(self) -> int:
+        return len(self.offsets)
+
+
+def dia_capacity(n: int, nnz: int, tile_rows: int = 512) -> int:
+    if n <= 0:
+        return 0
+    ndiag = min(_lib.DIA_MAX_DIAGONALS, (4 * nnz) // (3 * n))
+    return (n + tile_rows - 1) // tile_rows * tile_rows * ndiag
+
+
+def pack_many(matrices, pack: bool = True, dia: bool = False) -> None:
+    todo, todo_dia, seen = [], [], set()
     for m in matrices:
-        key = (m.col._version, m.val._version, m.col.data_ptr(), m.val.data_ptr())
-        if id(m) in seen or (m._packed is not None and m._packed_key == key):
+        if id(m) in seen:
             continue
         seen.add(id(m))
-        m._packed, m._packed_key = None, key
-        todo.append(m)
-    if not todo:
+        key = (m.col._version, m.val._version, m.col.data_ptr(), m.val.data_ptr())
+        if pack and not (m._packed is not None and m._packed_key == key):
+            m._packed, m._packed_key = None, key
+            todo.append(m)
+        if dia and not (m._dia is not None and m._dia_key == key):
+            m._dia, m._dia_key = None, key
+            todo_dia.append(m)
+    if not todo and not todo_dia:
         return
     lib = _lib.lib()
     tile_rows = int(lib.dp_csr_pack_tile_rows())
     by_device = {}
     for m in todo:
-        by_device.setdefault(m.device, []).append(m)
-    for dev, ms in by_device.items():
-        status = torch.zeros(len(ms), dtype=torch.int32, device=dev)
-        copies = []
+        by_device.setdefault(m.device, ([], []))[0].append(m)
+    for m in todo_dia:
+        by_device.setdefault(m.device, ([], []))[1].append(m)
+    for dev, (ms, ds) in by_device.items():
+        meta = _lib.DIA_META
+        status = torch.zeros(len(ms) + meta * len(ds), dtype=torch.int32, device=dev)
+        copies, dia_vals = [], []
         with torch.cuda.device(dev):
+            for j, m in enumerate(ds):
+                val = torch.empty(max(dia_capacity(m.n, m.nnz, tile_rows), 4), dtype=torch.float32, device=dev)
+                _lib.check(lib.dp_csr_dia(m.n, m.nnz, _lib.ptr(m.rowptr), _lib.ptr(m.col), _lib.ptr(m.val), _lib.ptr(val),
+                                          val.numel(), status.data_ptr() + 4 * (len(ms) + meta * j), _lib.stream_ptr(dev)),
+                           "dp_csr_dia")
+                dia_vals.append(val)
             for i, m in enumerate(ms):
                 nnz = m.nnz
                 col16 = torch.empty(max((nnz + 7) // 8 * 8, 8), dtype=torch.uint16, device=dev)
@@ -217,6 +253,12 @@
         verdicts = status.cpu().tolist()
         for m, pk, bad in zip(ms, copies, verdicts):
             m._packed = pk if bad == 0 else False
+        for j, (m, val) in enumerate(zip(ds, dia_vals)):
+            at = len(ms) + meta * j
+            bad, nd = verdicts[at], verdicts[at + 1]
+            ntiles = (m.n + tile_rows - 1) // tile_rows
+            m._dia = DiaCsr(val[: ntiles * nd * tile_rows].view(ntiles, nd, tile_rows), verdicts[at + 2: at + 2 + nd]) \
+                if bad == 0 else False
 
 
 def as_csr(matrix, device=None) -> CsrMatrix:
diff --git a/include/dpcg.h b/include/dpcg.h
--- a/include/dpcg.h
+++ b/include/dpcg.h
@@ -65,6 +65,11 @@
                 float* val32, int32_t* tile_base, int32_t* status_out, void* stream);
 int dp_spmv_csr_packed_f64(int32_t n, int32_t nnz, const int32_t* rowptr, const uint16_t* col16, const float* val32,
                            const int32_t* tile_base, const double* x, double* y, void* stream);
+
+#define DP_DIA_MAX_DIAGONALS 16
+#define DP_DIA_META (2 + 2 * DP_DIA_MAX_DIAGONALS)
+int dp_csr_dia(int32_t n, int32_t nnz, const int32_t* rowptr, const int32_t* col, const double* val, float* val_out,
+               int64_t capacity, int32_t* meta_out, void* stream);
 
 int dp_spmv_csr_f64(int32_t n, int32_t nnz, const int32_t* rowptr, const int32_t* col, const double* val,
                     const double* x, double* y, void* stream);
@@ -191,6 +196,25 @@
 int dp_pcg_solve_f64(const dp_pcg_system_t* systems_host, int32_t nsys, const dp_pcg_params_t* params_host,
                      int32_t* flag_out, void* workspace, size_t workspace_bytes, void* stream);
 
+typedef struct dp_dia {
+    const float* val;
+    int32_t ndiag;
+    int32_t off[DP_DIA_MAX_DIAGONALS];
+    int32_t reserved;
+} dp_dia_t;
+typedef struct dp_pcg_dia {
+    dp_dia_t a, m, mt;
+} dp_pcg_dia_t;
+
+int dp_pcg_solve_dia_f64(const dp_pcg_system_t* systems_host, const dp_pcg_dia_t* dia_host, int32_t nsys,
+                         const dp_pcg_params_t* params_host, int32_t* flag_out, void* workspace, size_t workspace_bytes,
+                         void* stream);
+#define DP_STREAM_F64 0
+#define DP_STREAM_PACKED 1
+#define DP_STREAM_DIA 2
+int dp_pcg_stream_format(const dp_pcg_system_t* systems_host, const dp_pcg_dia_t* dia_host, int32_t nsys,
+                         const dp_pcg_params_t* params_host);
+
 size_t dp_spconv_sort_workspace_bytes(int32_t batch_size, int32_t h);
 int dp_spconv_sort_sites(const int32_t* indices, int64_t nnz, int32_t batch_size, int32_t h, int32_t w, int32_t* rowptr,
                          int32_t* col, int32_t* perm, int32_t* flag_out, void* workspace, size_t workspace_bytes,
```

Measured after the change: 20.82 (median of 6 runs). +8.9%, better.
